# disanda/Deep-GAN-Encoders

Hardware: AMD Instinct MI355X
Metric: encoder-train images/sec (E_align_s2 step, StyleGAN2 FFHQ-1024) (higher is better)
Workload: dtype bf16; 1 GPU; E_align_s2 two-phase step, StyleGAN2-1024 G (train mode) + BE(startf=16, L=9) + LPIPS-VGG16 (seeded stand-in weights), batch 8/GPU; global_batch=8, img_size=1024, parallelism=dp1

## Files before the change

### deep-gan-encoders_amd/_lib.py

```python
import ctypes as C
import os

_HERE = os.path.dirname(os.path.abspath(__file__))
LIB_PATH = os.environ.get("DGE_LIB_PATH", os.path.join(_HERE, "libdge_hip.so"))


class DgeError(RuntimeError):
    pass


class ConvDesc(C.Structure):
    _fields_ = [
        ("x", C.c_void_p), ("w_packed", C.c_void_p), ("y", C.c_void_p), ("addend", C.c_void_p), ("dot_src", C.c_void_p),
        ("in_scale", C.c_void_p), ("in_shift", C.c_void_p), ("out_scale", C.c_void_p),
        ("bias", C.c_void_p), ("noise", C.c_void_p), ("noise_w", C.c_void_p), ("stats", C.c_void_p),
        ("B", C.c_int), ("H", C.c_int), ("W", C.c_int), ("Cin", C.c_int), ("Cout", C.c_int),
        ("ksize", C.c_int), ("up", C.c_int), ("in_s2d", C.c_int), ("noise_batch", C.c_int), ("noise_w_per_channel", C.c_int),
        ("act", C.c_int), ("bias_scale", C.c_float), ("gain", C.c_float), ("add_scale", C.c_float),
        ("dtype", C.c_int), ("in_up2", C.c_int), ("in_relu", C.c_int), ("stats_slots", C.c_int), ("w_layout", C.c_int),
        ("prep", C.c_int), ("prep_gain", C.c_float), ("prep_noise", C.c_void_p), ("prep_ns", C.c_void_p), ("prep_noise_batch", C.c_int),
        ("prep_stats", C.c_void_p), ("mask_relu", C.c_int), ("in_t2d", C.c_int),
        ("rgb_w", C.c_void_p), ("rgb_style", C.c_void_p), ("rgb_bias", C.c_void_p), ("rgb_out", C.c_void_p), ("rgb_wscale", C.c_float),
        ("rgb_skip_y", C.c_int), ("pool_out", C.c_int), ("pool_mask", C.c_void_p),
        ("prefetch_w", C.c_void_p), ("prefetch_ntot", C.c_int), ("prefetch_cin", C.c_int), ("in_bwd_coef", C.c_void_p),
        ("in_bwd_extra", C.c_void_p), ("in_bwd_extra_scale", C.c_float), ("fr_img4", C.c_void_p), ("fr_out", C.c_void_p),
    ]


class ConvPPDesc(C.Structure):
    _fields_ = [
        ("x", C.c_void_p), ("w_pp", C.c_void_p), ("y", C.c_void_p), ("w_bstride", C.c_longlong),
        ("out_scale", C.c_void_p), ("bias", C.c_void_p), ("noise", C.c_void_p), ("noise_w", C.c_void_p),
        ("B", C.c_int), ("H", C.c_int), ("W", C.c_int), ("Cin", C.c_int), ("Cout", C.c_int),
        ("noise_batch", C.c_int), ("noise_w_per_channel", C.c_int), ("act", C.c_int), ("bias_scale", C.c_float), ("gain", C.c_float),
        ("dgrad", C.c_int), ("in_s2d", C.c_int), ("stats_slots", C.c_int), ("prep", C.c_int), ("prep_noise_batch", C.c_int), ("mask_relu", C.c_int),
        ("in_t2d", C.c_int), ("add_scale", C.c_float), ("prep_gain", C.c_float),
        ("dot_src", C.c_void_p), ("addend", C.c_void_p), ("stats", C.c_void_p), ("prep_stats", C.c_void_p), ("prep_noise", C.c_void_p), ("prep_ns", C.c_void_p),
    ]


class DenseLayer(C.Structure):
    _fields_ = [("w", C.c_void_p), ("bias", C.c_void_p), ("I", C.c_int), ("O", C.c_int), ("wscale", C.c_float), ("bscale", C.c_float),
                ("add", C.c_float), ("act", C.c_int), ("gain", C.c_float)]


class S2GradEntry(C.Structure):
    _fields_ = [("P", C.c_void_p), ("st", C.c_void_p), ("d", C.c_void_p), ("s", C.c_void_p), ("bias", C.c_void_p), ("wsq", C.c_void_p),
                ("gs", C.c_void_p), ("wstyle", C.c_void_p),
                ("nslot_p", C.c_int), ("nslot_s", C.c_int), ("in_c", C.c_int), ("out_c", C.c_int), ("row", C.c_int), ("bscale", C.c_float)]


class SumPlanarEntry(C.Structure):
    _fields_ = [("partial", C.c_void_p), ("out", C.c_void_p), ("nslot", C.c_int), ("C", C.c_int), ("NS", C.c_int), ("pad", C.c_int)]


_P, _I, _F = C.c_void_p, C.c_int, C.c_float
SIGNATURES = {
    "dge_conv2d": [C.POINTER(ConvDesc), _P],
    "dge_fir_t2d": [_P, _P, _P, _I, _I, _I, _I, _I, _P],
    "dge_s2_style_grads": [C.POINTER(S2GradEntry), _I, _P, _I, _I, _I, _F, _P],
    "dge_conv_small_supported": [_I, _I, _I, _I, _I, _I, _I, _I],
    "dge_torgb_bwd_prep": [_P, _P, _P, _P, _P, _P, _I, _P, _P, _P, _I, _I, _I, _F, _F, _I, _P],
    "dge_demod_bwd_prep": [_P, _I, _P, _P, _P, _I, _I, _F, _P],
    "dge_sum_slots": [_P, _P, _I, _I, _I, _P],
    "dge_sum_slots_planar": [_P, _P, _I, _I, _I, _P],
    "dge_set_deterministic": [_I],
    "dge_get_deterministic": [],
    "dge_packed_n": [_I],
    "dge_pack_conv_weight": [_P, _P, _I, _I, _I, _I, _I, _F, _P],
    "dge_pack_conv_weights_multi": [_P, _P, _I, _I, _P],
    "dge_pack_desc_bytes": [],
    "dge_weight_sumsq": [_P, _P, _I, _I, _I, _F, _P],
    "dge_linear": [_P, _I, _P, _P, _P, _I, _I, _I, _I, _F, _F, _F, _I, _F, _I, _P],
    "dge_pixelnorm": [_P, _P, _I, _I, _F, _P],
    "dge_truncation": [_P, _P, _P, _I, _I, _I, _F, _I, _I, _P],
    "dge_torgb": [_P, _P, _P, _P, _P, _P, _I, _I, _I, _I, _F, _I, _P],
    "dge_conv_rgb_supported": [_I, _I, _I, _I, _I, _I, _I],
    "dge_conv_in_bwd_supported": [_I, _I, _I, _I, _I, _I, _I],
    "dge_conv_in_bwd_fromrgb_supported": [_I, _I, _I, _I, _I, _I, _I],
    "dge_conv_in_bwd_x_supported": [_I, _I, _I, _I, _I, _I, _I],
    "dge_conv_pool_supported": [_I, _I, _I, _I, _I, _I, _I],
    "dge_rgb_upsample_add": [_P, _P, _I, _I, _I, _P],
    "dge_nchw_to_nhwc": [_P, _P, _I, _I, _I, _I, _I, _P],
    "dge_nhwc_to_nchw": [_P, _P, _I, _I, _I, _I, _P],
    "dge_fromrgb": [_P, _P, _P, _P, _P, _I, _I, _I, _I, _P],
    "dge_fromrgb2": [_P, _P, _P, _P, _P, _P, _I, _I, _I, _I, _P],
    "dge_stats_finalize": [_P, _P, _P, _P, _I, _I, _I, _F, _P],
    "dge_stats_finalize_slots": [_P, _I, _P, _P, _P, _I, _I, _I, _F, _P],
    "dge_blend": [_P, _P, _P, _P, _P, _P, _I, _I, _I, _I, _I, _F, _F, _I, _P],
    "dge_loss_reduce": [_P, _P, _P, _I, _I, _I, _I, _I, _I, _I, _I, _P],
    "dge_crop_pool": [_P, _P, _I, _I, _I, _I, _I, _I, _I, _I, _P],
    "dge_ssim_fwd": [_P, _P, _P, _P, _I, _I, _I, _P],
    "dge_ssim_box7": [_P, _P, _P, _I, _I, _I, _F, _F, _F, _P],
    "dge_ssim_bwd": [_P, _P, _P, _P, _I, _I, _I, _F, _I, _P],
    "dge_space_loss_finalize": [_P, _P, _P, _P, _F, _F, _I, _P],
    "dge_space_loss_bwd": [_P, _P, _P, _P, _P, _I, _I, _I, _I, _I, _I, _I, _I, _F, _F, _I, _P],
    "dge_axpy_scalar": [_P, _P, _P, C.c_long, _F, _I, _P],
    "dge_lreq_adam_multi": [_I, _P, _P, _P, _P, _P, _F, _F, _P, _P, _P],
    "dge_modconv_bwd_prep": [_P, _P, _P, _P, _P, _P, _I, _I, _I, _I, _F, _I, _P],
    "dge_demod_bwd": [_P, _P, _P, _P, _P, _I, _I, _F, _P],
    "dge_linear_t": [_P, _I, _I, _P, _P, _P, _I, _I, _I, _I, _I, _F, _I, _P],
    "dge_torgb_bwd": [_P, _P, _P, _P, _P, _P, _I, _I, _I, _F, _I, _P],
    "dge_up2_bwd": [_P, _P, _I, _I, _I, _P],
    "dge_conv_wgrad": [_P, _P, _P, _P, _P, _I, _I, _I, _I, _I, _I, _I, _P],
    "dge_act_bwd": [_P, _P, _P, _P, _P, _I, _I, _I, _I, _I, _I, _F, _F, _I, _P],
    "dge_in_bwd_coef": [_P, _P, _P, _P, _P, _P, _I, _I, _I, _P],
    "dge_in_bwd_coef_slots": [_P, _I, _P, _P, _P, _P, _P, _I, _I, _I, _P],
    "dge_in_bwd": [_P, _P, _P, _P, _P, _P, _P, _I, _I, _I, _I, _I, _F, _I, _I, _P],
    "dge_chan_sum": [_P, _P, _I, _I, _I, _F, _I, _P],
    "dge_fromrgb_bwd": [_P, _P, _P, _P, _I, _I, _I, _I, _P],
    "dge_head_entry_size": [],
# ... 31 lines not shown
    "dge_upconv_fir": [_P, _P, _P, _P, _P, _P, _I, _P, _I, _P, _F, _F, _I, _I, _I, _I, _I, _I, _I, _P],
    "dge_cbn_affine": [_P, _P, _I, _P, _P, _F, _P, _P, _I, _I, _P],
    "dge_slice_up": [_P, _P, _I, _I, _I, _I, _I, _I, _I, _P],
    "dge_attention": [_P, _P, _P, _P, _I, _I, _I, _I, _I, _I, _P],
    "dge_rgb_tanh": [_P, _P, _I, _I, _I, _I, _P],
    "dge_guided_relu_bwd": [_P, _P, _P, C.c_long, _I, _I, _P],
    "dge_maxpool2_relu_bwd": [_P, _P, _P, _I, _I, _I, _I, _I, _I, _P],
    "dge_maxpool2_bwd_relu": [_P, _P, _P, _P, _I, _I, _I, _I, _I, _P],
    "dge_adaptive_pool7": [_P, _P, _I, _I, _I, _I, _I, _P],
    "dge_adaptive_pool7_bwd": [_P, _P, _I, _I, _I, _I, _I, _P],
    "dge_class_target": [_P, _P, _P, _P, _I, _I, _P],
    "dge_gather_row": [_P, _P, _P, _I, _I, _F, _P],
    "dge_campp_map": [_P, _P, _P, _P, _P, _I, _I, _I, _I, _I, _P],
    "dge_cam_resize": [_P, _P, _P, _I, _I, _I, _I, _I, _P],
    "dge_mask2cam_blocks": [_I],
    "dge_mask2cam": [_P, _P, _P, _P, _P, _P, _P, _I, _I, _P],
    "dge_randn": [_P, _I, _P, _P, _P, _P, C.c_ulonglong, _P, _P],
    "dge_version": [],
    "dge_env_reload": [],
    "dge_blend_pool_mask": [_P, _P, _P, _P, _P, _I, _I, _I, _I, _F, _F, _I, _P],
    "dge_act_bwd_mask": [_P, _P, _P, _P, _P, _I, _I, _I, _I, _I, _F, _F, _I, _P],
    "dge_loss_reduce3": [_P, _P, _P, _I, _I, _I, _I, _P, _I, _P],
    "dge_crop_pool_multi": [_P, _P, _P, _P, _I, _I, _I, _I, _P],
    "dge_space_loss_bwd3": [_P, _P, _P, _P, _P, _I, _I, _I, _P, _P, _P, _P, _I, _P],
    "dge_space_loss_bwd_split": [_P, _P, _P, _P, _P, _I, _I, _I, _P, _P, _P, _P, _I, _P],
    "dge_in_bwd_fromrgb": [_P, _P, _P, _I, _P, _P, _P, _P, _I, _P, _P, _P, _I, _I, _I, _I, _I, _F, _I, _P],
    "dge_in_bwd_fused": [_P, _P, _P, _I, _P, _P, _P, _P, _I, _P, _P, _P, _P, _I, _I, _I, _I, _I, _F, _I, _I, _P],
    "dge_sum_slots_planar_multi": [C.POINTER(SumPlanarEntry), _I, _P],
    "dge_heads_fwd": [_P, _I, _P, _P, _I, _I, _I, _P],
    "dge_conv_pp_supported": [_I, _I, _I, _I, _I, _I],
    "dge_pack_conv_pp": [_P, _P, _I, _I, _F, _P, _P, _F, _I, _I, _P],
    "dge_dense_chain": [_P, _I, C.POINTER(DenseLayer), _I, _P, _I, _I, _I, _F, _P],
    "dge_conv_wgrad_dots": [_P, _P, _P, _P, _P, _P, _P, _I, _I, _I, _I, _I, _I, _I, _P],
    "dge_pack_conv_pp_rows": [_P, _I, _P, _I, _I, _P, _I, _P, _F, _I, _I, _P],
    "dge_conv_pp": [C.POINTER(ConvPPDesc), _P],
    "dge_up_pp_supported": [_I, _I, _I, _I, _I, _I],
    "dge_pack_up_pp": [_P, _P, _I, _I, _P, _P, _F, _I, _P],
    "dge_up_pp": [_P, _P, C.c_longlong, _P, _P, _I, _P, _P, _F, _F, _I, _I, _I, _I, _I, _I, _P],
    "dge_latent_pnorm_fwd": [_P, _P, _P, C.c_long, _I, _P],
    "dge_latent_pnorm_bwd": [_P, _P, _P, _P, C.c_long, _I, _F, _P],
    "dge_wplus_lerp": [_P, _P, _I, _F, _P, _I, _I, _I, _P],
    "dge_wplus_lerp_bwd": [_P, _F, _P, C.c_long, _I, _P],
    "dge_embed_track": [_P, _P, _P, C.c_long, _P, _P, _P, _P, _P, _I, _I, _I, _F, _F, _P],
    "dge_mapping_bwd": [_P, _I, C.POINTER(DenseLayer), _I, _P, _P, _I, _P, _P, _I, _I, _I, _F, _P],
}

_lib = None


def lib():
    global _lib
    if _lib is None:
        if not os.path.exists(LIB_PATH):
            raise DgeError(f"{LIB_PATH} is missing: build it with deep-gan-encoders_amd/csrc/build.sh "
                           "(__graft_entry__.build()). There is no fallback path.")
        _lib = C.CDLL(LIB_PATH)
        for name, args in SIGNATURES.items():
            fn = getattr(_lib, name)
            fn.argtypes = args
            fn.restype = C.c_int
        for name in ("dge_last_error", "dge_last_kernel"):
            getattr(_lib, name).restype = C.c_char_p
            getattr(_lib, name).argtypes = []
        if os.environ.get("DGE_DETERMINISTIC") == "1":
            import torch
            if torch.cuda.is_available() and _lib.dge_set_deterministic(1) != 0:
# ... 12 lines not shown
```

### deep-gan-encoders_amd/autograd_enc_bwd.py

```python
import os

import torch

from . import ops
from .autograd_enc import grads_in_order, heads_layout, linear_backward
from .weight_cache import pack_cache, packed

FUSE_IN_BWD = not os.environ.get("DGE_NO_FUSED_IN_BWD")


def encoder_backward(E, saved, g_w):
    if saved is None:
        raise RuntimeError("encoder forward ran without saved activations")
    cache = pack_cache(E)
    dev = g_w.device
    L = E.layer_count
    B = g_w.shape[0]
    grads = {}
    g_out = fr = None
    later = ops.DeferredSums()
    post = []

    def flush_sums():
        later.flush()
        for f in post:
            f()
        post.clear()
    R = saved["img"].shape[2]
    dt = ops.dtype_of(saved["x0"])
    heads = None
    if saved.get("musig_all") is not None:
        lay = heads_layout(E, B, dev)
        if g_w.stride(2) != 1 or g_w.stride(1) != lay["O"]:
            g_w = g_w.contiguous()
        f32 = dict(dtype=torch.float32, device=dev)
        gms_all, gw_all = torch.empty(lay["total_m"], **f32), torch.empty(lay["total_w"], **f32)
        gb_all = torch.empty(lay["n"] * lay["O"], **f32)
        ops.check(ops.lib().dge_heads_bwd(ops._p(lay["tab"]), lay["n"], lay["max_I"], ops._f32(g_w), g_w.stride(0),
                                          ops._f32(saved["musig_all"]), ops._p(gms_all), ops._p(gw_all), ops._p(gb_all), B, lay["O"],
                                          ops._stream()), "dge_heads_bwd")

        def heads(i, name):
            moff, woff, boff, I = lay["items"][i]
            grads[name + ".weight"] = gw_all[woff:woff + lay["O"] * I].view(lay["O"], I)
            grads[name + ".bias"] = gb_all[boff:boff + lay["O"]]
            return gms_all[moff:moff + B * I].view(B, I)
    for j in range(L - 1, -1, -1):
        blk = E.decode_block[j]
        rec = saved["blocks"][j]
        pre = f"decode_block.{j}."
        Cc, C2 = blk.inputs, blk.outputs
        H = R >> j
        N = H * H
        last = not blk.has_last_conv
        has3 = Cc != C2
        g_w2, g_w1 = g_w[:, 2 * (L - 1 - j)], g_w[:, 2 * (L - 1 - j) + 1]
        if heads is not None:
            gms2, gms1 = heads(2 * j + 1, pre + "inver_mod2"), heads(2 * j, pre + "inver_mod1")
        else:
            gms2 = linear_backward(blk.inver_mod2, g_w2, rec["musig2"], grads, pre + "inver_mod2")
            gms1 = linear_backward(blk.inver_mod1, g_w1, rec["musig1"], grads, pre + "inver_mod1")
        x, x1 = rec["x"], rec["x1"]
        extra, extra_pool, extra_scale = None, False, 1.0
        fuse2 = False
        if not last:
            if g_out is None:
                raise RuntimeError("non-final encoder block without an output gradient")
            red2 = ops.zeros((3 if has3 else 2, C2), dev)
            g_pre2 = ops.act_bwd_mask(g_out, rec["m2"], rec["n2"], scale=0.111 * 0.25, red=red2, planar=True, defer=later)
            grads[pre + "bias_2"] = red2[0].reshape(1, C2, 1, 1)
            grads[pre + "noise_weight_2"] = red2[1].reshape(1, C2, 1, 1)
            gW2 = ops.zeros(tuple(blk.conv_2.weight.shape), dev)
            dots2 = ops.SlotStats(B, Cc, dev)
            fuse2 = FUSE_IN_BWD and ops.conv_in_bwd_supported(B, H, H, C2, Cc, dt) and \
                ops.conv_wgrad_dots(g_pre2, x1, gW2, rec["sc2"], rec["sh2"], blk.conv_2.weight, dots2)
            if not fuse2:
                ops.conv_wgrad(g_pre2, x1, gW2, rec["sc2"], rec["sh2"])
            grads[pre + "conv_2.weight"] = gW2
            if not fuse2:
                g_y2 = ops.conv2d(g_pre2, packed(cache, blk.conv_2, dt, ops.PACK_DGRAD, H), Cc, 3, stats=dots2, dot_src=x1)
            if has3:
                post.append(lambda n=pre + "conv_3.bias", t=red2[2]: grads.__setitem__(n, t * 0.889))
                gW3 = ops.zeros(tuple(blk.conv_3.weight.shape), dev)
                ops.conv_wgrad(g_out, rec["xp"], gW3)
                grads[pre + "conv_3.weight"] = ops.scale_(gW3, 0.889)
                extra = ops.conv2d(g_out, packed(cache, blk.conv_3, dt, ops.PACK_DGRAD), Cc, 1, gain=0.889)
                extra_pool, extra_scale = True, 0.25
            else:
                extra, extra_pool, extra_scale = g_out, True, 0.889 * 0.25
        else:
            if g_out is not None:
                raise RuntimeError("the final encoder block's activation output carries no gradient in E_align")
            g_y2, dots2 = None, None
        coef2 = (dots2, gms2, rec["musig2"], rec["sc2"], rec["sh2"], N)
        red1 = ops.zeros((2, Cc), dev)
        if fuse2:
            redp = ops.SlotStats(B, Cc, dev)
            g_pre1 = ops.conv2d(g_pre2, packed(cache, blk.conv_2, dt, ops.PACK_DGRAD, H), Cc, 3, dot_src=x1,
                                in_bwd=dict(coef=ops.in_bwd_coef(*coef2), noise=rec["n1"].reshape(B, H, H), red=redp))
            ops._sum_planar(redp.buf.view(-1, Cc, 2), red1, later)
        else:
            g_pre1 = ops.in_bwd(g_y2, x1, coef2, noise=rec["n1"], act=True, red=red1, planar=True, defer=later)
        grads[pre + "bias_1"] = red1[0].reshape(1, Cc, 1, 1)
        grads[pre + "noise_weight_1"] = red1[1].reshape(1, Cc, 1, 1)
        gW1 = ops.zeros(tuple(blk.conv_1.weight.shape), dev)
        dots1 = ops.SlotStats(B, Cc, dev)
        fuse_fr = FUSE_IN_BWD and j == 0 and saved.get("img4") is not None and ops.conv_in_bwd_fromrgb_supported(B, H, H, Cc, Cc, dt) and \
            ops.conv_wgrad_dots(g_pre1, x, gW1, rec["sc1"], rec["sh1"], blk.conv_1.weight, dots1)
        fuse_x = FUSE_IN_BWD and not fuse_fr and j > 0 and (extra is None or extra_pool) and ops.conv_in_bwd_x_supported(B, H, H, Cc, Cc, dt) and \
            ops.conv_wgrad_dots(g_pre1, x, gW1, rec["sc1"], rec["sh1"], blk.conv_1.weight, dots1)
        if not (fuse_fr or fuse_x):
            ops.conv_wgrad(g_pre1, x, gW1, rec["sc1"], rec["sh1"])
        grads[pre + "conv_1.weight"] = gW1
        coef1 = (dots1, gms1, rec["musig1"], rec["sc1"], rec["sh1"], N)
        if fuse_fr:
            frh = ops.SlotStats(B, Cc, dev)
            ops.conv2d(g_pre1, packed(cache, blk.conv_1, dt, ops.PACK_DGRAD, H), Cc, 3, dot_src=x, out=x.new_empty((1, 1, 1, 1)),
                       in_bwd=dict(coef=ops.in_bwd_coef(*coef1), fr=frh, img4=saved["img4"], extra=extra if extra_pool else None,
                                   extra_scale=extra_scale))
            fr = ops._sum_planar(frh.buf.view(-1, Cc, 4), torch.empty((4, Cc), dtype=torch.float32, device=dev), later)
        elif fuse_x:
            g_out = ops.conv2d(g_pre1, packed(cache, blk.conv_1, dt, ops.PACK_DGRAD, H), Cc, 3, dot_src=x,
                               in_bwd=dict(coef=ops.in_bwd_coef(*coef1), extra=extra, extra_scale=extra_scale))
        else:
            g_y1 = ops.conv2d(g_pre1, packed(cache, blk.conv_1, dt, ops.PACK_DGRAD, H), Cc, 3, stats=dots1, dot_src=x)
        if fuse_fr or fuse_x:
            pass
        elif j == 0 and Cc <= 512:
            fr = ops.in_bwd_fromrgb(g_y1, x, coef1, saved["img"].float(), extra=extra, extra_pool=extra_pool, extra_scale=extra_scale,
                                    defer=later)
        else:
            g_out = ops.in_bwd(g_y1, x, coef1, extra=extra, extra_pool=extra_pool, extra_scale=extra_scale)
# ... 13 lines not shown
```

### deep-gan-encoders_amd/csrc/capi.hip

```cpp
#include <stdarg.h>
#include <stdio.h>
#include "common.h"
#include "conv_params.h"
#include "../../include/dge_hip.h"

static thread_local char g_err[512] = "";
void dge_set_error(const char* fmt, ...) {
    va_list ap; va_start(ap, fmt); vsnprintf(g_err, sizeof(g_err), fmt, ap); va_end(ap);
}
extern "C" const char* dge_last_error(void) { return g_err; }
static thread_local char g_kernel[160] = "";
void dge_note_kernel(const char* fmt, ...) {
    va_list ap; va_start(ap, fmt); vsnprintf(g_kernel, sizeof(g_kernel), fmt, ap); va_end(ap);
}
extern "C" const char* dge_last_kernel(void) { return g_kernel; }
extern "C" int dge_version(void) { return 100; }

#include <vector>
static std::vector<void (*)(const DgeDet*)>& det_setters() { static std::vector<void (*)(const DgeDet*)> v; return v; }
void dge_det_register(void (*setter)(const DgeDet*)) { det_setters().push_back(setter); }
static DgeDet g_det_host = {0, nullptr, nullptr, 0, 0};
int dge_det_upload_failed = 0;
bool dge_det_fits(long long ndomains, long long nslots, long long L) {
    return !g_det_host.enabled || (ndomains * nslots * L <= g_det_host.ws_floats && ndomains <= (long long)g_det_host.ncounters);
// ... 62 lines not shown
    p.x = d->x; p.w = d->w_packed; p.y = d->y; p.addend = d->addend; p.dot_src = d->dot_src;
    p.in_scale = d->in_scale; p.in_shift = d->in_shift; p.out_scale = d->out_scale;
    p.bias = d->bias; p.noise = d->noise; p.noise_w = d->noise_w; p.stats = d->stats;
    p.B = d->B; p.H = d->H; p.W = d->W; p.Cin = d->Cin; p.Cout = d->Cout;
    p.Ntot_valid = d->up ? 4 * d->Cout : d->Cout;
    p.Ntot = dge_packed_n(p.Ntot_valid);
    p.up = d->up; p.in_s2d = d->in_s2d; p.in_up2 = d->in_up2; p.in_relu = d->in_relu;
    const int OH = d->up ? 2 * d->H : d->H, OW = d->up ? 2 * d->W : d->W;
    p.noise_bstride = d->noise_batch > 1 ? OH * OW : 0;
    p.noise_w_stride = d->noise_w_per_channel ? 1 : 0;
    p.act = d->act; p.bias_scale = d->bias_scale; p.gain = d->gain; p.add_scale = d->add_scale;
    p.tiles_x = p.tiles_y = 0;
    p.w_frag = d->w_layout == 1 ? 1 : 0;
    p.prep = d->prep ? 1 : 0;
    p.mask_relu = d->mask_relu ? 1 : 0;
    p.in_t2d = d->in_t2d ? 1 : 0;
    DGE_CHECK(!d->in_t2d || (d->ksize == 3 && !d->up && !d->in_s2d && !d->in_up2 && !d->in_scale && !d->in_shift && d->w_layout == 0),
              "conv2d: in_t2d is a plain 3x3 launch (no other read mode, no prologue affine, row-major weights)");
    p.prep_gain = d->prep_gain; p.prep_noise = d->prep_noise; p.prep_ns = d->prep_ns; p.prep_stats = d->prep_stats;
    p.prep_noise_bstride = d->prep_noise_batch > 1 ? OH * OW : 0;
    DGE_CHECK(!d->prep || (d->dot_src && d->prep_stats && d->prep_gain > 0.f && !d->up), "conv2d: prep needs dot_src, prep_stats, a positive prep_gain and no up mode");
    DGE_CHECK(!d->prep || !dge_get_deterministic(), "conv2d: the fused tail backward (prep) is not offered in deterministic mode; run dge_modconv_bwd_prep");
    DGE_CHECK(d->w_layout == 0 || d->w_layout == 1, "conv2d: bad w_layout %d", d->w_layout);
    p.stats_slots = d->stats_slots > 0 ? d->stats_slots : 1;
    p.rgb_w = d->rgb_out ? d->rgb_w : nullptr; p.rgb_style = d->rgb_style; p.rgb_bias = d->rgb_bias; p.rgb_out = d->rgb_out;
    p.rgb_wscale = d->rgb_wscale; p.rgb_skip_y = (d->rgb_out && d->rgb_skip_y) ? 1 : 0;
    p.pool_out = d->pool_out ? 1 : 0; p.pool_mask = d->pool_out ? (unsigned*)d->pool_mask : nullptr;
    const bool pf = d->w_layout == 1 && d->prefetch_w && d->prefetch_ntot >= 64 && d->prefetch_ntot % 64 == 0 &&
                    (d->prefetch_cin == 512 || d->prefetch_cin == 256);
    p.pf_w = pf ? d->prefetch_w : nullptr; p.pf_ntot = pf ? d->prefetch_ntot : 0; p.pf_cin = pf ? d->prefetch_cin : 0;
    p.in_coef = d->in_bwd_coef;
    p.in_extra = d->in_bwd_coef ? d->in_bwd_extra : nullptr; p.in_extra_scale = d->in_bwd_extra_scale;
    p.fr_img4 = d->in_bwd_coef ? d->fr_img4 : nullptr; p.fr_out = d->in_bwd_coef ? d->fr_out : nullptr;
    if (d->in_bwd_coef) {
        DGE_CHECK(!dge_get_deterministic(), "conv2d: in_bwd_coef is not offered in deterministic mode; run dge_in_bwd");
        DGE_CHECK(d->ksize == 3 && !d->up && dge_conv_stream_eligible(p, d->dtype, d->ksize), "conv2d: in_bwd_coef is offered where "
                  "dge_conv_in_bwd_supported() says so, with dot_src and prep_stats, without stats / prep");
    }
    if (d->pool_out)
        DGE_CHECK(!d->up && dge_conv_pool_ok(p, d->dtype, d->ksize), "conv2d: the pooled epilogue is offered where dge_conv_pool_supported() "
                  "says so (conv_2 of the first encoder blocks on the streaming kernel)");
    if (d->rgb_out) {
        DGE_CHECK(d->rgb_w && d->rgb_style && d->rgb_bias, "conv2d: rgb_out needs rgb_w, rgb_style, rgb_bias");
        DGE_CHECK(dge_conv_rgb_ok(p, d->dtype, d->ksize), "conv2d: the fused toRGB is offered where dge_conv_rgb_supported() says so "
                  "(bf16 3x3 32 -> 32 launches of the streaming kernel)");
    }
    return dge_conv_launch(p, d->dtype, d->ksize, s);
}

extern "C" int dge_conv_pool_supported(int B, int H, int W, int Cin, int Cout, int ksize, int dtype) {
    ConvParams p = {};
    p.B = B; p.H = H; p.W = W; p.Cin = Cin; p.Cout = Cout; p.Ntot_valid = Cout; p.Ntot = dge_packed_n(Cout);
    p.in_shift = (const float*)16; p.noise_w_stride = 1;
    return dge_conv_pool_ok(p, dtype, ksize) ? 1 : 0;
}

extern "C" int dge_conv_in_bwd_supported(int B, int H, int W, int Cin, int Cout, int ksize, int dtype) {
    ConvParams p = {};
    p.B = B; p.H = H; p.W = W; p.Cin = Cin; p.Cout = Cout; p.Ntot_valid = Cout; p.Ntot = dge_packed_n(Cout);
    p.dot_src = (const void*)16; p.prep_stats = (float*)16; p.in_coef = (const float*)16;
    return (ksize == 3 && !dge_get_deterministic() && dge_conv_stream_eligible(p, dtype, ksize)) ? 1 : 0;
}
extern "C" int dge_conv_in_bwd_x_supported(int B, int H, int W, int Cin, int Cout, int ksize, int dtype) {
    ConvParams p = {};
    p.B = B; p.H = H; p.W = W; p.Cin = Cin; p.Cout = Cout; p.Ntot_valid = Cout; p.Ntot = dge_packed_n(Cout);
    p.dot_src = (const void*)16; p.in_coef = (const float*)16;
    return (ksize == 3 && !dge_get_deterministic() && dge_conv_stream_eligible(p, dtype, ksize)) ? 1 : 0;
}
extern "C" int dge_conv_in_bwd_fromrgb_supported(int B, int H, int W, int Cin, int Cout, int ksize, int dtype) {
    ConvParams p = {};
    p.B = B; p.H = H; p.W = W; p.Cin = Cin; p.Cout = Cout; p.Ntot_valid = Cout; p.Ntot = dge_packed_n(Cout);
    p.dot_src = (const void*)16; p.in_coef = (const float*)16; p.fr_img4 = (const float*)16; p.fr_out = (float*)16;
    return (ksize == 3 && !dge_get_deterministic() && dge_conv_stream_eligible(p, dtype, ksize)) ? 1 : 0;
}

extern "C" int dge_conv_rgb_supported(int B, int H, int W, int Cin, int Cout, int ksize, int dtype) {
    ConvParams p = {};
    p.B = B; p.H = H; p.W = W; p.Cin = Cin; p.Cout = Cout; p.Ntot_valid = Cout; p.Ntot = dge_packed_n(Cout);
    return dge_conv_rgb_ok(p, dtype, ksize) ? 1 : 0;
}

__global__ void sum_slots_kernel(const float* __restrict__ partial, float* __restrict__ out, int nslot, int n, int accumulate) {
    const int i = blockIdx.x * blockDim.x + threadIdx.x;
    if (i >= n) return;
    float s = 0.f;
    int k = 0;
    for (; k + 8 <= nslot; k += 8) {
        float v[8];
#pragma unroll
        for (int j = 0; j < 8; j++) v[j] = partial[(size_t)(k + j) * n + i];
#pragma unroll
        for (int j = 0; j < 8; j++) s += v[j];
    }
    for (; k < nslot; k++) s += partial[(size_t)k * n + i];
// ... 61 lines not shown
```

### deep-gan-encoders_amd/csrc/conv_params.h

```cpp
#pragma once
#include <hip/hip_runtime.h>

struct ConvParams {
    const void* x;
    const void* w;
    void* y;
    const void* addend;
    const void* dot_src;
    const float* in_scale;
    const float* in_shift;
    const float* out_scale;
    const float* bias;
    const float* noise;
    const float* noise_w;
    float* stats;
    int stats_slots;
    int B, H, W, Cin, Cout;
    int Ntot;
    int Ntot_valid;
    int up;
    int in_s2d;
    int in_relu;
    int in_up2;
    int noise_bstride;
    int noise_w_stride;
    int act;
    float bias_scale, gain, add_scale;
    int tiles_x, tiles_y;
    int dbg;
    int w_frag;
    int prep;
    float prep_gain;
    const float* prep_noise;
    const float* prep_ns;
    int prep_noise_bstride;
    float* prep_stats;
    int mask_relu;
    int in_t2d;
    const float* rgb_w;
    const float* rgb_style;
    const float* rgb_bias;
    float* rgb_out;
    float rgb_wscale;
    int rgb_skip_y;
    int pool_out;
    unsigned* pool_mask;
    const void* pf_w;
    int pf_ntot, pf_cin;
    const float* in_coef;
    const void* in_extra; float in_extra_scale; const float* fr_img4; float* fr_out;
};

int dge_conv_launch(const ConvParams& p, int dtype, int ksize, hipStream_t s);
extern "C" int dge_conv_ntile(int ntot);

bool dge_conv_stream_eligible(const ConvParams& p, int dtype, int ksize);
int dge_conv_stream_launch(const ConvParams& p, hipStream_t s);
bool dge_conv_rgb_ok(const ConvParams& p, int dtype, int ksize);
bool dge_conv_pool_ok(const ConvParams& p, int dtype, int ksize);
bool dge_conv_small_shape_ok(int H, int W, int cin, int ntot, int ksize, int in_s2d, int in_up2, int dtype);
int dge_conv_small_launch(const ConvParams& p, hipStream_t s);
bool dge_conv_pw_eligible(const ConvParams& p, int dtype, int ksize);
int dge_conv_pw_launch(const ConvParams& p, hipStream_t s);
```

### deep-gan-encoders_amd/csrc/conv_stream.hip

```cpp
#include <type_traits>
#include "common.h"
#include <stdlib.h>
#include "conv_params.h"

namespace {

typedef __attribute__((ext_vector_type(4))) unsigned rsrc_t;
#define DGE_LDS " lds\n\t"

__device__ __forceinline__ unsigned rfl(unsigned v) { return __builtin_amdgcn_readfirstlane(v); }
__device__ __forceinline__ unsigned lds_off(const void* p) {
    return (unsigned)(size_t)(const __attribute__((address_space(3))) unsigned char*)p;
}
constexpr int ilog2(int v) { return v <= 1 ? 0 : 1 + ilog2(v >> 1); }

__device__ __forceinline__ rsrc_t make_rsrc(unsigned long long base, unsigned bytes) {
    rsrc_t r;
    r[0] = rfl((unsigned)base); r[1] = rfl((unsigned)(base >> 32) & 0xffffu); r[2] = rfl(bytes); r[3] = 0x00020000u;
    return r;
}

#define DGE_P(off) "buffer_load_dwordx4 %1, %3, 0 offen offset:" #off " lds\n\t"
#define DGE_PB(off) "buffer_load_dwordx4 %4, %3, 0 offen offset:" #off " lds\n\t"
#define DGE_M0 "s_mov_b32 m0, %2\n\ts_nop 0\n\t"
// ... 9 lines not shown
        if (wave == 0) asm volatile(DGE_M0 DGE_P(0) : "=&s"(keep) : "v"(voff), "s"(m0v), "s"(rs) : "memory");
        else asm volatile(DGE_M0 DGE_MASK(0xf) DGE_P(1024) DGE_UNMASK : "=&s"(keep) : "v"(voff), "s"(m0v), "s"(rs) : "memory");
    } else if constexpr (CIN == 32 && TEAM == 1) {
        asm volatile(DGE_M0 DGE_P(0) DGE_P(1024) DGE_MASK(0xff) DGE_P(2048) DGE_UNMASK : "=&s"(keep) : "v"(voff), "s"(m0v), "s"(rs) : "memory");
    } else if constexpr (CIN == 32 && TEAM == 2) {
        if (wave == 0) asm volatile(DGE_M0 DGE_P(0) DGE_MASK(0xff) DGE_P(2048) DGE_UNMASK : "=&s"(keep) : "v"(voff), "s"(m0v), "s"(rs) : "memory");
        else asm volatile(DGE_M0 DGE_P(1024) "s_mov_b32 m0, %5\n\ts_nop 0\n\tbuffer_load_dwordx4 %1, %4, 0 offen lds"
                          : "=&s"(keep) : "v"(voff), "s"(m0v), "s"(rs), "s"(rs_null), "s"(m0_dummy) : "memory");
    } else if constexpr (CIN == 64 && TEAM == 1) {
        asm volatile(DGE_M0 DGE_P(0) DGE_PB(1024) DGE_P(2048) DGE_PB(3072)
                     "s_mov_b32 m0, %6\n\t" DGE_MASK(0xffff) "buffer_load_dwordx4 %5, %3, 0 offen lds\n\t" DGE_UNMASK
                     : "=&s"(keep) : "v"(voff), "s"(m0v), "s"(rs), "v"(voff_b), "v"(voff_c), "s"(m0v + 4096u) : "memory");
    } else {
        if (wave == 0)
            asm volatile(DGE_M0 DGE_P(0) DGE_P(2048)
                         "s_mov_b32 m0, %5\n\t" DGE_MASK(0xffff) "buffer_load_dwordx4 %4, %3, 0 offen lds\n\t" DGE_UNMASK
                         : "=&s"(keep) : "v"(voff), "s"(m0v), "s"(rs), "v"(voff_c), "s"(m0v + 4096u) : "memory");
        else
            asm volatile(DGE_M0 DGE_P(1024) DGE_P(3072) "s_mov_b32 m0, %5\n\ts_nop 0\n\tbuffer_load_dwordx4 %1, %4, 0 offen lds"
                         : "=&s"(keep) : "v"(voff_b), "s"(m0v), "s"(rs), "s"(rs_null), "s"(m0_dummy) : "memory");
    }
}
__device__ __forceinline__ void dma_piece(unsigned voff, rsrc_t rs, unsigned m0v) {
    asm volatile("s_mov_b32 m0, %1\n\ts_nop 0\n\tbuffer_load_dwordx4 %0, %2, 0 offen lds" : : "v"(voff), "s"(m0v), "s"(rs) : "memory");
}
template <int NP> __device__ __forceinline__ void dma_dot(unsigned voff, unsigned voff1, rsrc_t rs, unsigned m0v) {
    if constexpr (NP == 1)
        asm volatile("s_mov_b32 m0, %1\n\ts_nop 0\n\tbuffer_load_dwordx4 %0, %2, 0 offen lds" : : "v"(voff), "s"(m0v), "s"(rs) : "memory");
    else
        asm volatile("s_mov_b32 m0, %1\n\ts_nop 0\n\tbuffer_load_dwordx4 %0, %2, 0 offen lds\n\t"
                     "buffer_load_dwordx4 %3, %2, 0 offen offset:1024 lds" : : "v"(voff), "s"(m0v), "s"(rs), "v"(voff1) : "memory");
}

enum { FL_GEN = 0, FL_ENC = 1, FL_ENC_STATS = 2, FL_DOT = 3, FL_DOT_PREP = 4, FL_GEN_RGB = 5, FL_ENC_POOL = 6, FL_DOT_IN = 7, FL_DOT_FR = 8, FL_DOT_INX = 9 };

template <int CIN, int COUT, int FL>
struct SC {
    static constexpr int PXB = CIN * 2, CH = PXB / 16, LOGCH = ilog2(CH), KS = CIN / 16;
    static constexpr int TEAM = COUT == 64 ? 2 : 1;
    static constexpr int TPW = 4 / TEAM;
    static constexpr int MT = COUT / 32 > 0 ? COUT / 32 : 1;
    static constexpr int MTW = MT / TEAM;
    static constexpr int HW = 34, RB = HW * PXB;
    static constexpr int PIECES = (RB + 1023) / 1024;
    static constexpr bool PREP = FL == FL_DOT_PREP, RGB = FL == FL_GEN_RGB, POOL = FL == FL_ENC_POOL, FRB = FL == FL_DOT_FR, INX = FL == FL_DOT_INX, INB = FL == FL_DOT_IN || FRB || INX;
    static_assert(!RGB || COUT == 32 || (COUT == 64 && TEAM == 2), "fused toRGB: 32 output channels per wave, one wave or a 2-wave team per pixel");
    static constexpr bool DOT = FL == FL_DOT || PREP || INB, STATS = FL == FL_ENC_STATS, ENC = FL == FL_ENC || FL == FL_ENC_STATS || POOL;
    static constexpr bool NOISE = !DOT || PREP || (INB && !FRB && !INX);
    static constexpr int NR = 6;
    static constexpr int dot_depth(int nr) { for (int d = 4; d >= 1; d--) if (d <= nr - 3 && nr % (d + 1) == 0) return d; return 1; }
    static constexpr int D = DOT ? dot_depth(6) : 2;
    static constexpr int DR = DOT ? D + 1 : NR;
    static_assert(NR % DR == 0, "dot ring period");
    static constexpr int CPB = COUT * 2;
    static constexpr int CW = COUT / TEAM >= 32 ? 32 : 16;
    static constexpr int DCH = CW * MTW * 2 / 16;
    static constexpr int LOGDCH = ilog2(DCH);
    static constexpr int DROWB = 32 * DCH * 16, DPIECES = DROWB / 1024;
    static_assert(!DOT || MTW == 1, "data-gradient mode: one M tile per wave");
    static constexpr int XPW = TEAM == 2 ? (PIECES + 1) / 2 : PIECES;
    static constexpr int LPR = XPW + (DOT ? DPIECES : 0) + (FRB ? 2 : 0) + (INX ? 1 : 0);
    static constexpr int X_OFF = 0;
    static constexpr int XRING = NR * RB;
    static constexpr int N_OFF = (XRING + 1023) / 1024 * 1024;
    static constexpr int NRING = NOISE ? 2048 : 0;
    static_assert(NR <= 8, "a noise piece holds 8 rows");
    static constexpr int D_OFF = N_OFF + TEAM * NRING;
    static constexpr int DRING = DOT ? DR * DROWB : 0;
    static constexpr int E_OFF = D_OFF + TEAM * DRING;
    static constexpr int ERING = FRB ? 2 * DR * 512 : (INX ? DR * 1024 : 0);
    static_assert(!INX || (CIN == COUT && CIN >= 32), "block-input flavour: 32 -> 32, 64 -> 64");
    static_assert(!FRB || (CIN == 16 && COUT == 16 && TEAM == 1), "FromRGB reduction flavour: 16 -> 16");
    static constexpr int T_OFF = E_OFF + TEAM * ERING;
    static constexpr int TBYTES = 32 * MTW * 16 * 4;
    static constexpr int DUMMY_OFF = T_OFF + TEAM * TBYTES;
    static constexpr int RGBX_OFF = DUMMY_OFF + (TEAM == 2 ? 1024 : 0);
    static constexpr int LDS_BYTES = RGBX_OFF + (RGB && TEAM == 2 ? 1024 : 0);
    static constexpr int NEED = 4 * 9 * KS * MTW + 32 * MTW + 16 + (ENC ? 16 * MTW : 0) + (STATS || DOT ? 32 * MTW : 0) + (DOT ? 16 : 0) + (PREP ? 16 : 0) + (RGB ? 11 : 0) + (POOL ? 20 * MTW : 0) + 36;
    static constexpr int WPE = ((PREP || INB) && CIN == 64) ? 1 : (NEED <= 128 ? 4 : (NEED <= 168 ? 3 : 2));
    static_assert(D <= NR - 3, "the slot of the row being fetched must be dead");
    static_assert((D - 1) * LPR + 1 < 64, "vmcnt range");
};

template <int LOGC> __device__ __forceinline__ int chunk_swz(int px) { return (px >> (4 - LOGC)) & ((1 << LOGC) - 1); }

template <int CW> __device__ __forceinline__ int chan_of_row(int m) {
    const int j = m >> 3, k = (m >> 2) & 1, i = m & 3;
    if (CW == 16) return j < 2 ? 8 * k + 4 * j + i : -1;
    return 16 * (j >> 1) + 8 * k + 4 * (j & 1) + i;
}

template <int CIN, int COUT, int FL>
__global__ __launch_bounds__((64 * SC<CIN, COUT, FL>::TEAM * SC<CIN, COUT, FL>::TPW), (SC<CIN, COUT, FL>::WPE))
void conv_stream_kernel(ConvParams p, int nstrips, int nseg, int seg_rows, int njobs, int jobs_per_xcd) {
    using C = SC<CIN, COUT, FL>;
    extern __shared__ __attribute__((aligned(1024))) unsigned char lds_all[];
#ifdef DGE_SC_TIMING
    const long long tj0 = __builtin_readcyclecounter();
#endif
    const int lane = threadIdx.x & 63;
    const int wid = (int)rfl(threadIdx.x >> 6);
    const int team = wid / C::TEAM;
    const int wave = wid % C::TEAM;
    unsigned char* __restrict__ lds = lds_all + team * C::LDS_BYTES;
    const unsigned lds0 = lds_off(lds_all) + team * C::LDS_BYTES;
    const int n31 = lane & 31, kh = lane >> 5;

    int job = ((blockIdx.x & 7) * jobs_per_xcd + (blockIdx.x >> 3)) * C::TPW + team;
    if ((blockIdx.x >> 3) >= jobs_per_xcd || job >= njobs) return;
    const int strip = job % nstrips; job /= nstrips;
    const int seg = job % nseg;
    const int b = job / nseg;
    const int x0 = strip * 32;
    const int r0 = seg * seg_rows;
// ... 10 lines not shown
    const unsigned long long DOTb = C::DOT ? (unsigned long long)p.dot_src + (unsigned long long)b * p.H * yrow_bytes : Xb;

    unsigned voff, voff_b = 0, voff_c = 0;
    {
        const int px = lane >> C::LOGCH, cs = lane & (C::CH - 1);
        const int gx = x0 - 1 + px;
        voff = (unsigned)(gx * C::PXB + ((cs ^ chunk_swz<C::LOGCH>(px)) << 4));
        if constexpr (CIN == 64) {
            voff_b = (unsigned)(gx * C::PXB + ((cs ^ chunk_swz<C::LOGCH>(px + 8)) << 4));
            voff_c = voff + 4096;
        }
    }
    const unsigned nvoff = (unsigned)(((lane >> 3) * p.W + x0 + (lane & 7) * 4) * 4);
    unsigned dvoff = 0, dvoff1 = 0;
    if constexpr (C::DOT) {
        const int px = lane >> C::LOGDCH, cs = lane & (C::DCH - 1);
        const int chunk0 = wave * 4;
        dvoff = (unsigned)((x0 + px) * C::CPB + ((chunk0 + (cs ^ chunk_swz<C::LOGDCH>(px))) << 4));
        constexpr int PPP = 64 / C::DCH;
        dvoff1 = (unsigned)((x0 + px + PPP) * C::CPB + ((chunk0 + (cs ^ chunk_swz<C::LOGDCH>(px + PPP))) << 4)) - 1024u;
    }
    const rsrc_t rs_null = make_rsrc(Xb, 0);
    const unsigned exrow_bytes = (C::FRB || C::INX) ? (unsigned)(p.W >> 1) * C::CPB : 0u, imrow_bytes = C::FRB ? (unsigned)p.W * 16u : 0u;
    const unsigned long long EXb = ((C::FRB || C::INX) && p.in_extra) ? (unsigned long long)p.in_extra + (unsigned long long)b * (p.H >> 1) * exrow_bytes : Xb;
    const unsigned long long IMb = C::FRB ? (unsigned long long)p.fr_img4 + (unsigned long long)b * p.H * imrow_bytes : Xb;
    const unsigned evoff = C::INX ? (unsigned)(((x0 >> 1) + (lane >> 2)) * C::CPB + wave * 64 + (((lane & 3) ^ chunk_swz<2>(lane >> 2)) << 4))
                                  : (unsigned)((x0 >> 1) * 32 + (lane & 31) * 16);
    const unsigned ivoff = (unsigned)((x0 + (lane & 31)) * 16);

    unsigned long long xptr = Xb + (unsigned long long)(long long)(r0 - 1) * xrow_bytes;
    unsigned long long dptr = DOTb + (unsigned long long)(long long)(r0 - 2) * yrow_bytes;
    auto issue = [&](int h, int slot, int slot_d) {
        const int gy = r0 - 1 + h;
        const bool xv = (unsigned)gy < (unsigned)p.H && h <= rows + 1;
        const rsrc_t rx = make_rsrc(xptr, xv ? xrow_bytes : 0u);
        xptr += xrow_bytes;
        const unsigned m0x = lds0 + C::X_OFF + slot * C::RB;
        dma_row<CIN, C::TEAM>(wave, voff, voff_b, voff_c, rx, rs_null, m0x, lds0 + C::DUMMY_OFF);
        const bool ov = h >= 2 && h <= rows + 1;
        if constexpr (C::DOT) {
            const rsrc_t rd = make_rsrc(dptr, ov ? yrow_bytes : 0u);
            dptr += yrow_bytes;
            dma_dot<C::DPIECES>(dvoff, dvoff1, rd, lds0 + C::D_OFF + wave * C::DRING + slot_d * C::DROWB);
        }
        if constexpr (C::INX) {
            const int oy = gy - 1;
            const rsrc_t re = make_rsrc(EXb + (unsigned long long)(ov ? (oy >> 1) : 0) * exrow_bytes, (ov && p.in_extra) ? exrow_bytes : 0u);
            dma_piece(evoff, re, lds0 + C::E_OFF + wave * C::ERING + slot_d * 1024);
        }
        if constexpr (C::FRB) {
            const int oy = gy - 1;
            const rsrc_t re = make_rsrc(EXb + (unsigned long long)(ov ? (oy >> 1) : 0) * exrow_bytes, (ov && p.in_extra) ? exrow_bytes : 0u);
            const rsrc_t ri = make_rsrc(IMb + (unsigned long long)(ov ? oy : 0) * imrow_bytes, ov ? imrow_bytes : 0u);
            unsigned long long keep;
            asm volatile(DGE_MASK(0xffffffff) "s_mov_b32 m0, %2\n\ts_nop 0\n\tbuffer_load_dwordx4 %1, %3, 0 offen lds\n\t"
                         "s_mov_b32 m0, %4\n\ts_nop 0\n\tbuffer_load_dwordx4 %5, %6, 0 offen lds\n\t" DGE_UNMASK
                         : "=&s"(keep) : "v"(evoff), "s"(lds0 + C::E_OFF + slot_d * 512), "s"(re), "s"(lds0 + C::E_OFF + C::DR * 512 + slot_d * 512), "v"(ivoff), "s"(ri) : "memory");
        }
    };
    auto issue_noise = [&](int q, unsigned buf_off) {
        const int gy = r0 + q;
        const bool v = nzsrc != nullptr && gy < p.H && q < rows;
        const rsrc_t rn = make_rsrc(NZb + (unsigned long long)(v ? gy : 0) * nzrow_bytes, v ? (unsigned)(p.H - gy) * nzrow_bytes : 0u);
        dma_piece(nvoff, rn, lds0 + C::N_OFF + wave * C::NRING + buf_off);
    };
    asm volatile("s_waitcnt vmcnt(0)" ::: "memory");
    if constexpr (C::NOISE) issue_noise(0, 0u);
    StaticFor<C::D + 2>::run([&](auto hc) { constexpr int h = decltype(hc)::value; issue(h, h % C::NR, (h + C::NR - 2) % C::NR % C::DR); });

    uint4 wf[C::MTW][9][C::KS];
    float* __restrict__ TT = (float*)(lds + C::T_OFF + wave * C::TBYTES);
    {
        const bf16_t* __restrict__ Wp = (const bf16_t*)p.w;
        float sc[C::KS][8], rt[C::KS][8];
#pragma unroll
        for (int ks = 0; ks < C::KS; ks++) {
            const int k0 = ks * 16 + kh * 8;
#pragma unroll
            for (int e = 0; e < 8; e++) {
                sc[ks][e] = p.in_scale ? p.in_scale[b * CIN + k0 + e] : 1.f;
                const float sh = (C::ENC && p.in_shift) ? p.in_shift[b * CIN + k0 + e] : 0.f;
                rt[ks][e] = sc[ks][e] != 0.f ? sh / sc[ks][e] : 0.f;
            }
        }
#pragma unroll
        for (int mt = 0; mt < C::MTW; mt++) {
            const int cl = chan_of_row<C::CW>(n31);
            const int o = (wave * C::MTW + mt) * 32 + cl;
            const bool ov = cl >= 0 && o < COUT;
            float osc = p.gain;
            if (!C::DOT && p.out_scale && ov) osc *= p.out_scale[b * COUT + o];
            if (C::INB && ov) osc *= p.in_coef[((size_t)b * COUT + o) * 3];
            const int oc = ov ? o : 0;
            float c_bias = (!C::DOT && p.bias) ? p.bias[oc] : 0.f;
            float c_nw = (C::NOISE && p.noise) ? p.noise_w[oc * p.noise_w_stride] : 0.f;
            float c_osc = (C::DOT && !C::INB && p.out_scale) ? p.out_scale[b * COUT + oc] : 1.f;
            float c_in1 = 0.f, c_in2 = 0.f;
            if constexpr (C::INB) { c_in1 = p.in_coef[((size_t)b * COUT + oc) * 3 + 1]; c_in2 = p.in_coef[((size_t)b * COUT + oc) * 3 + 2]; }
            float tall = 0.f, tleft = 0.f, tright = 0.f;
            {
// ... 120 lines not shown

    const int gx = x0 + n31;
    const bool pv = gx < p.W;
    const unsigned yoff = (unsigned)gx * C::CPB + (unsigned)(wave * C::MTW * 32 * 2) + kh * 16;
    const bool pool_lane = C::POOL && (n31 & 1) == 0 && pv;
    const unsigned py_voff = pool_lane ? (unsigned)(gx >> 1) * C::CPB + (unsigned)(wave * C::MTW * 64) + kh * 16 : 0x80000000u;
    const unsigned pm_voff = pool_lane ? ((unsigned)(gx >> 1) * (COUT / 8) + (unsigned)(wave * C::MTW * 4) + kh) * 4u : 0x80000000u;
    const unsigned pool_px = C::POOL ? (unsigned)(p.H >> 1) * (unsigned)(p.W >> 1) : 0u;
    const __amdgpu_buffer_rsrc_t rs_pool = __builtin_amdgcn_make_buffer_rsrc((unsigned char*)p.y + (size_t)b * pool_px * C::CPB, 0, (int)(pool_px * C::CPB), 0x00020000);
    const __amdgpu_buffer_rsrc_t rs_mask = __builtin_amdgcn_make_buffer_rsrc((C::POOL && p.pool_mask) ? (unsigned char*)p.pool_mask + (size_t)b * pool_px * (COUT / 8) * 4 : (unsigned char*)p.y, 0,
                                                                               (C::POOL && p.pool_mask) ? (int)(pool_px * (COUT / 8) * 4) : 0, 0x00020000);

    float s0[C::MTW][(C::STATS || C::DOT) ? 16 : 1], s1[C::MTW][(C::STATS || C::DOT) ? 16 : 1], s2[(C::PREP || C::INB) ? 16 : 1];
    if constexpr (C::STATS || C::DOT) {
#pragma unroll
        for (int mt = 0; mt < C::MTW; mt++)
#pragma unroll
            for (int r = 0; r < 16; r++) { s0[mt][r] = 0.f; s1[mt][r] = 0.f; }
    }
    if constexpr (C::PREP || C::INB) {
#pragma unroll
        for (int r = 0; r < 16; r++) s2[r] = 0.f;
    }
    float prow[C::POOL ? C::MTW : 1][C::POOL ? 16 : 1];
    unsigned psign[C::POOL ? C::MTW : 1];
    const float pg_pos = p.prep_gain, pg_neg = 0.2f * p.prep_gain, pz_pos = 1.f / p.prep_gain, pz_neg = 1.f / (0.2f * p.prep_gain);
    const float pns = (C::PREP && p.prep_noise && p.prep_ns) ? p.prep_ns[0] : 0.f;
    const float fr_es = (C::FRB || C::INX) ? p.in_extra_scale : 0.f;

#define DGE_T(k)
    auto step = [&](auto ic, int s, unsigned npar) {
        constexpr int I = decltype(ic)::value;
        DGE_T(0);
        constexpr int NAFTER = (C::D - 1) * C::LPR + ((C::NOISE && I >= 1 && I <= C::D - 1) ? 1 : 0);
        asm volatile("s_waitcnt vmcnt(%0)" :: "i"(NAFTER) : "memory");
        if constexpr (C::RGB && C::TEAM == 2) asm volatile("s_waitcnt lgkmcnt(0)" ::: "memory");
        if constexpr (C::TEAM == 2) __builtin_amdgcn_s_barrier();
        if constexpr (C::RGB && C::TEAM == 2) { if (wave == 0 && s > 0) rgb_flush(s - 1); }
        DGE_T(1);
        if constexpr (C::NOISE && I == 0) issue_noise(s + C::NR, npar ^ 1024u);
        issue(s + 2 + C::D, (I + 2 + C::D) % C::NR, (I + C::D) % C::DR);
        DGE_T(2);

        const int gy = r0 + s;
        constexpr int NQ = 9 * C::KS;
        constexpr int PF = NQ < 6 ? NQ : 6;
        auto frag_addr = [&](auto qc) {
            constexpr int q = decltype(qc)::value;
            constexpr int tap = q / C::KS, ks = q % C::KS, dy = tap / 3, dx = tap % 3;
            return loff[dx][ks] + (unsigned)(((I + dy) % C::NR) * C::RB);
        };
        float nz = 0.f;
        if constexpr (C::NOISE) nz = lds_f(nzoff + npar + I * 128);
        uint4 bq[PF];
        StaticFor<PF>::run([&](auto qc) { bq[decltype(qc)::value] = lds_u4(frag_addr(qc)); });
        f32x16_t acc[C::MTW];
        StaticFor<NQ>::run([&](auto qc) {
            constexpr int q = decltype(qc)::value;
            constexpr int tap = q / C::KS, ks = q % C::KS;
            const bf16x8_t bf = *(const bf16x8_t*)&bq[q % PF];
#pragma unroll
            for (int mt = 0; mt < C::MTW; mt++) {
                acc[mt] = __builtin_amdgcn_mfma_f32_32x32x16_bf16(*(const bf16x8_t*)&wf[mt][tap][ks], bf, q == 0 ? ((C::DOT && !C::INB) ? zero16 : biasv[mt]) : acc[mt], 0, 0, 0);
            }
            if constexpr (q + PF < NQ) bq[q % PF] = lds_u4(frag_addr(std::integral_constant<int, q + PF>{}));
        });

        __builtin_amdgcn_sched_group_barrier(0x100, PF + (C::NOISE ? 1 : 0), 0);
        StaticFor<NQ - PF>::run([&](auto) {
            __builtin_amdgcn_sched_group_barrier(0x008, C::MTW, 0);
            __builtin_amdgcn_sched_group_barrier(0x100, 1, 0);
        });
        __builtin_amdgcn_sched_group_barrier(0x008, PF * C::MTW, 0);
// ... 130 lines not shown
            if constexpr (C::RGB) {
                f32x16_t t = __builtin_amdgcn_mfma_f32_32x32x16_bf16(*(const bf16x8_t*)&rgbA[0], *(const bf16x8_t*)&o0, zero16, 0, 0, 0);
                t = __builtin_amdgcn_mfma_f32_32x32x16_bf16(*(const bf16x8_t*)&rgbA[1], *(const bf16x8_t*)&o1, t, 0, 0, 0);
                if constexpr (C::TEAM == 2) {
                    if (wave == 0) { rgbh[0] = t[0] + t[4] + rgbb[0]; rgbh[1] = t[1] + t[5] + rgbb[1]; rgbh[2] = t[2] + t[6] + rgbb[2]; }
                    else if (kh == 0) {
                        const unsigned a = lds0 + C::RGBX_OFF + (unsigned)(s & 1) * 384 + n31 * 4;
                        *(lds_wfp)(a) = t[0] + t[4]; *(lds_wfp)(a + 128) = t[1] + t[5]; *(lds_wfp)(a + 256) = t[2] + t[6];
                    }
                } else if (kh == 0 && pv) {
                    float* __restrict__ ro = p.rgb_out + ((size_t)b * 3 * p.H + gy) * p.W + gx;
                    const size_t plane = (size_t)p.H * p.W;
                    ro[0] = t[0] + t[4] + rgbb[0]; ro[plane] = t[1] + t[5] + rgbb[1]; ro[2 * plane] = t[2] + t[6] + rgbb[2];
                }
                if (p.rgb_skip_y) continue;
            }
            if (full_strip) {
                *(uint4*)dst = o0;
                if constexpr (NREG == 16) *(uint4*)(dst + 32) = o1;
            } else if (pv) {
                *(uint4*)dst = o0;
                if constexpr (NREG == 16) *(uint4*)(dst + 32) = o1;
            }
        }
        DGE_T(4);
    };

#ifdef DGE_SC_TIMING
    const int tjob_id = ((blockIdx.x & 7) * jobs_per_xcd + (blockIdx.x >> 3)) * C::TPW + team;
    __builtin_amdgcn_sched_barrier(0);
    const long long tj1 = __builtin_readcyclecounter();
    __builtin_amdgcn_sched_barrier(0);
#endif
    unsigned npar = 0;
    for (int s0_ = 0; s0_ < rows; s0_ += C::NR, npar ^= 1024u) {
        bool done = false;
        StaticFor<C::NR>::run([&](auto ic) {
            constexpr int I = decltype(ic)::value;
            if (!done) {
                if ((C::POOL && (I & 1)) || s0_ + I < rows) step(ic, s0_ + I, npar);
                else done = true;
            }
        });
    }
    if constexpr (C::RGB && C::TEAM == 2) {
        asm volatile("s_waitcnt lgkmcnt(0)" ::: "memory");
        __builtin_amdgcn_s_barrier();
        if (wave == 0 && rows > 0) rgb_flush(rows - 1);
    }
    asm volatile("s_waitcnt vmcnt(0)" ::: "memory");
#ifdef DGE_SC_TIMING
    if (lane == 0 && wave == 0) {
        long long* tl = (long long*)p.y + (size_t)tjob_id * 4;
        tl[0] = tj0; tl[1] = tj1; tl[2] = __builtin_readcyclecounter(); tl[3] = ((long long)rows << 40) | (long long)(__builtin_amdgcn_s_memrealtime() & 0xffffffffffll);
    }
#endif

    if constexpr (C::FRB) {
        float va = 0.f, vc = 0.f;
#pragma unroll
        for (int r = 0; r < 16; r++) {
            float a = pv ? s0[0][r] : 0.f, c = pv ? s1[0][r] : 0.f;
#pragma unroll
            for (int m = 1; m < 32; m <<= 1) { a += __shfl_xor(a, m, 64); c += __shfl_xor(c, m, 64); }
            if (n31 == r) { va = a; vc = c; }
        }
// ... 37 lines not shown
                }
            }
            if (!C::PREP && !C::INB && det && det_arrive_wave(b, nseg * nstrips * C::TEAM)) {
                for (int idx = lane; idx < COUT * 2; idx += 64)
                    p.stats[(size_t)b * COUT * 2 + idx] = det_sum(b, nseg * nstrips, COUT * 2, idx);
            }
        }
    }
}

template <int CIN, int COUT, int FL>
int launch_stream(const ConvParams& p0, hipStream_t s) {
    using C = SC<CIN, COUT, FL>;
    ConvParams p = p0;
    auto kern = conv_stream_kernel<CIN, COUT, FL>;
    static int caps[16] = {0};
    int dev = 0;
    (void)hipGetDevice(&dev);
    int& cap = caps[dev >= 0 && dev < 16 ? dev : 0];
    if (!cap) {
        (void)hipFuncSetAttribute((const void*)kern, hipFuncAttributeMaxDynamicSharedMemorySize, C::LDS_BYTES * C::TPW);
        int occ = 0, ncu = 256;
        (void)hipDeviceGetAttribute(&ncu, hipDeviceAttributeMultiprocessorCount, dev);
        if (hipOccupancyMaxActiveBlocksPerMultiprocessor(&occ, (const void*)kern, 64 * C::TEAM * C::TPW, C::LDS_BYTES * C::TPW) != hipSuccess || occ < 1) occ = 1;
        cap = occ * ncu * C::TPW;
    }
    const int nstrips = (p.W + 31) / 32;
    int nseg = cap / (p.B * nstrips);
    if (dge_env().stream_nseg > 0) nseg = dge_env().stream_nseg;
    int maxseg = p.H / 16; if (maxseg < 1) maxseg = 1;
    if (nseg > maxseg) nseg = maxseg;
    if (nseg < 1) nseg = 1;
    int seg_rows = (p.H + nseg - 1) / nseg;
    if (C::POOL) seg_rows += seg_rows & 1;
    nseg = (p.H + seg_rows - 1) / seg_rows;
    const int njobs = p.B * nstrips * nseg;
    const int nwg = (njobs + C::TPW - 1) / C::TPW;
    const int jobs_per_xcd = (nwg + 7) / 8;
    const char* fl = FL == FL_GEN ? "gen" : (FL == FL_ENC ? "enc" : (FL == FL_ENC_STATS ? "enc_stats" : (FL == FL_DOT ? "dot" : (FL == FL_DOT_PREP ? "dot_prep" : (FL == FL_GEN_RGB ? "gen_rgb" : (FL == FL_DOT_IN ? "dot_in" : (FL == FL_DOT_FR ? "dot_fromrgb" : (FL == FL_DOT_INX ? "dot_inx" : "enc_pool"))))))));
    dge_note_kernel("conv_stream<bf16,%d,%d,%s>", CIN, COUT, fl);
    hipLaunchKernelGGL(kern, dim3((unsigned)(jobs_per_xcd * 8)), dim3(64 * C::TEAM * C::TPW), C::LDS_BYTES * C::TPW, s, p, nstrips, nseg, seg_rows, njobs, jobs_per_xcd);
    DGE_LAUNCH_CHECK("conv_stream");
    return 0;
}

template <int CIN, int COUT>
int launch_flavour(const ConvParams& p, hipStream_t s) {
    if (p.in_coef && p.fr_out) {
        if constexpr (CIN == 16 && COUT == 16) return launch_stream<CIN, COUT, FL_DOT_FR>(p, s);
        dge_set_error("conv_stream: the FromRGB reduction epilogue is built for 16 -> 16 only");
        return -1;
    }
    if (p.in_coef && !p.prep_stats) {
        if constexpr (CIN == COUT && CIN >= 32) return launch_stream<CIN, COUT, FL_DOT_INX>(p, s);
        dge_set_error("conv_stream: the block-input instance-norm backward epilogue is built for 32 -> 32 and 64 -> 64 only");
        return -1;
    }
    if (p.in_coef) {
        if constexpr ((CIN == 32 && COUT == 16) || (CIN == 64 && COUT == 32)) return launch_stream<CIN, COUT, FL_DOT_IN>(p, s);
        dge_set_error("conv_stream: the instance-norm backward epilogue is built for 32 -> 16 and 64 -> 32 only");
        return -1;
    }
    if (p.dot_src) {
        if constexpr (CIN == COUT && CIN >= 32) {
            if (p.prep) return launch_stream<CIN, COUT, FL_DOT_PREP>(p, s);
        }
        if (p.prep) { dge_set_error("conv_stream: the fused tail backward is built for 32->32 and 64->64 only"); return -1; }
        return launch_stream<CIN, COUT, FL_DOT>(p, s);
    }
    const bool enc = p.stats || p.in_shift || (p.noise && p.noise_w_stride != 0);
    if (p.rgb_out) {
        if constexpr ((CIN == 32 && COUT == 32) || (CIN == 64 && COUT == 64)) { if (!enc) return launch_stream<CIN, COUT, FL_GEN_RGB>(p, s); }
        dge_set_error("conv_stream: the fused toRGB is built for the generator flavour of 32 -> 32 and 64 -> 64 only");
        return -1;
    }
    if (p.pool_out) {
        if constexpr ((CIN == 16 && COUT == 32) || (CIN == 32 && COUT == 64)) { if (!p.stats) return launch_stream<CIN, COUT, FL_ENC_POOL>(p, s); }
        dge_set_error("conv_stream: the pooled epilogue is built for the encoder's 16 -> 32 and 32 -> 64 layers without statistics");
        return -1;
    }
    if constexpr (CIN == 64) {
        if (enc) { dge_set_error("conv_stream: encoder flavour with Cin = 64 is not built"); return -1; }
    } else {
        if (p.stats) return launch_stream<CIN, COUT, FL_ENC_STATS>(p, s);
        if (enc) return launch_stream<CIN, COUT, FL_ENC>(p, s);
    }
    return launch_stream<CIN, COUT, FL_GEN>(p, s);
}

}

bool dge_conv_stream_eligible(const ConvParams& p, int dtype, int ksize) {
    if (dtype != DGE_BF16 || ksize != 3 || p.up || p.in_s2d || p.in_up2 || p.in_relu || p.addend || p.mask_relu || p.in_t2d) return false;
    if (!(p.Cin == 16 || p.Cin == 32 || p.Cin == 64) || !(p.Cout == 16 || p.Cout == 32 || p.Cout == 64)) return false;
    if (p.W % 4 != 0 || p.W < 64 || p.H < 32) return false;
    if ((long)p.H * p.W < 128L * 128) return false;
    {
        const long px = (long)p.B * p.H * p.W;
        const bool enc = p.stats || p.in_shift || (p.noise && p.noise_w_stride != 0);
        if (!dge_env().force_stream) {
            if (!p.dot_src && px < (enc ? (1L << 20) : (1L << 18))) return false;
            if (p.dot_src && px < (1L << 16)) return false;
        }
    }
    if ((long)p.W * p.Cin * 2 >= (1L << 31) || (long)p.H * p.W * 64 * 2 >= (1L << 40)) return false;
    if (p.dot_src && !p.stats && !p.in_coef) return false;
    if (p.in_coef && !p.fr_out && p.prep_stats && !(p.dot_src && !p.prep && !p.stats && ((p.Cin == 32 && p.Cout == 16) || (p.Cin == 64 && p.Cout == 32)))) return false;
    if (p.in_coef && !p.fr_out && !p.prep_stats && !(p.dot_src && !p.prep && !p.stats && p.Cin == p.Cout && p.Cin >= 32 && p.H % 2 == 0 && p.W % 2 == 0)) return false;
    if (p.fr_out && !(p.in_coef && p.dot_src && p.fr_img4 && !p.prep && !p.stats && p.Cin == 16 && p.Cout == 16 && p.H % 2 == 0 && p.W % 2 == 0)) return false;
    if (p.prep && !(p.Cin == p.Cout && p.Cin >= 32)) return false;
    if (p.Cin == 64 && !p.dot_src && (p.stats || p.in_shift || (p.noise && p.noise_w_stride != 0))) return false;
    if (p.dot_src && (p.bias || p.noise || p.in_shift || p.act != DGE_ACT_NONE)) return false;
    if (p.noise && p.noise_w == nullptr) return false;
    if (dge_env().no_stream) return false;
    return true;
}

bool dge_conv_pool_ok(const ConvParams& p, int dtype, int ksize) {
    return ((p.Cin == 16 && p.Cout == 32) || (p.Cin == 32 && p.Cout == 64)) && !p.dot_src && !p.stats && !p.rgb_out && p.H % 2 == 0 && p.W % 2 == 0 &&
           dge_conv_stream_eligible(p, dtype, ksize);
}

bool dge_conv_rgb_ok(const ConvParams& p, int dtype, int ksize) {
    return ((p.Cin == 32 && p.Cout == 32) || (p.Cin == 64 && p.Cout == 64)) && !p.dot_src && !p.stats && !p.in_shift && !(p.noise && p.noise_w_stride != 0) &&
           dge_conv_stream_eligible(p, dtype, ksize);
}

int dge_conv_stream_launch(const ConvParams& p, hipStream_t s) {
#define GO(CI, CO) if (p.Cin == CI && p.Cout == CO) return launch_flavour<CI, CO>(p, s)
#ifdef DGE_SC_ONLY
#define GO2(...) GO(__VA_ARGS__)
    GO2(DGE_SC_ONLY);
#undef GO2
#else
    GO(16, 16); GO(16, 32); GO(16, 64); GO(32, 16); GO(32, 32); GO(32, 64); GO(64, 16); GO(64, 32); GO(64, 64);
#endif
#undef GO
    dge_set_error("conv_stream: unsupported channel configuration %d -> %d", p.Cin, p.Cout);
    return -1;
}
```

### deep-gan-encoders_amd/csrc/enc_bwd_kernels.hip

```cpp
#include <stdlib.h>
#include "common.h"
#include "../../include/dge_hip.h"

template <int NTAP>
__device__ __forceinline__ void wgrad_flush(const f32x16_t (&acc)[NTAP], float* smem, float* __restrict__ dW, int o0, int i0,
                                            int Co, int Ci, int tid, int lane, int wave) {
    float* red = smem;
    float* stage = smem + 4096;
#pragma unroll
    for (int t = 0; t < NTAP; t++) {
        __syncthreads();
#pragma unroll
        for (int r = 0; r < 16; r++) red[wave * 1024 + r * 64 + lane] = acc[t][r];
        __syncthreads();
#pragma unroll
        for (int q = 0; q < 4; q++) {
            const int e = tid + q * 256;
            const int r = e >> 6, ln = e & 63;
            const int ol = (r & 3) + 8 * (r >> 2) + 4 * (ln >> 5), il = ln & 31;
            stage[(ol * 32 + il) * NTAP + t] = (red[e] + red[1024 + e]) + (red[2048 + e] + red[3072 + e]);
        }
    }
    __syncthreads();
    const int ni = (Ci - i0 < 32 ? Ci - i0 : 32) * NTAP;
// ... 289 lines not shown
                                                       float* __restrict__ red_out, int H, int W, int C, int pool, float scale, float slope) {
    constexpr int EP = Elem<T>::PER16;
    __shared__ float red[256 * NS * EP];
    const int b = blockIdx.y;
    const int cpt = C / EP, ppi = 256 / cpt;
    const int chunk = threadIdx.x % cpt, slot = threadIdx.x / cpt;
    const int HW = H * W, UW = pool ? W / 2 : W, UHW = pool ? HW / 4 : HW;
    const float raw_w = pool ? 0.25f : 1.f;
    float s[NS][EP];
#pragma unroll
    for (int k = 0; k < NS; k++)
#pragma unroll
        for (int e = 0; e < EP; e++) s[k][e] = 0.f;
    for (int p0 = blockIdx.x * ppi; p0 < HW; p0 += gridDim.x * ppi) {
        const int p = p0 + slot;
        if (slot < ppi && p < HW) {
            const int q = pool ? (p / W / 2) * UW + (p % W) / 2 : p;
            float g[EP], av[EP];
            unpack16(*(const uint4*)(gup + ((size_t)b * UHW + q) * C + chunk * EP), g, (T*)nullptr);
            unpack16(*(const uint4*)(a + ((size_t)b * HW + p) * C + chunk * EP), av, (T*)nullptr);
            const float nz = noise ? noise[(size_t)b * HW + p] : 0.f;
#pragma unroll
            for (int e = 0; e < EP; e++) {
                if constexpr (NS == 3) s[2][e] += raw_w * g[e];
                g[e] = scale * g[e] * (av[e] > 0.f ? 1.f : slope);
                s[0][e] += g[e]; s[1][e] += g[e] * nz;
            }
            *(uint4*)(gpre + ((size_t)b * HW + p) * C + chunk * EP) = pack16(g, (T*)nullptr);
        }
    }
    if (red_out) block_chan_flush<EP, NS>(s, cpt, ppi, red_out + (size_t)b * C * NS, C, red);
}

template <typename T, int NS>
__global__ __launch_bounds__(256) void act_bwd_mask_kernel(const T* __restrict__ gup, const unsigned* __restrict__ mask,
                                                            const float* __restrict__ noise, T* __restrict__ gpre,
                                                            float* __restrict__ red_out, int H, int W, int C, float scale, float slope) {
    constexpr int EP = Elem<T>::PER16;
    __shared__ float red[256 * NS * EP];
    const int b = blockIdx.y;
    const int cpt = C / EP, ppi = 256 / cpt;
    const int chunk = threadIdx.x % cpt, slot = threadIdx.x / cpt;
    const int UW = W / 2, UHW = (H / 2) * UW, HW = H * W;
    float s[NS][EP];
#pragma unroll
    for (int k = 0; k < NS; k++)
#pragma unroll
        for (int e = 0; e < EP; e++) s[k][e] = 0.f;
    const int stride = gridDim.x * ppi;
    for (int q0 = blockIdx.x * ppi; q0 < UHW; q0 += 2 * stride) {
        const int qq[2] = {q0 + slot, q0 + slot + stride};
        bool ok[2]; uint4 gv[2]; unsigned mv[2]; int p00[2]; float nzv[2][4];
#pragma unroll
        for (int h = 0; h < 2; h++) {
            ok[h] = slot < ppi && qq[h] < UHW;
            gv[h] = make_uint4(0, 0, 0, 0); mv[h] = 0; p00[h] = 0;
#pragma unroll
            for (int c4 = 0; c4 < 4; c4++) nzv[h][c4] = 0.f;
            if (ok[h]) {
                gv[h] = *(const uint4*)(gup + ((size_t)b * UHW + qq[h]) * C + chunk * EP);
                mv[h] = mask[((size_t)b * UHW + qq[h]) * cpt + chunk];
                const int oy = qq[h] / UW, ox = qq[h] - oy * UW;
                p00[h] = (2 * oy) * W + 2 * ox;
                if (noise) {
#pragma unroll
                    for (int c4 = 0; c4 < 4; c4++) nzv[h][c4] = noise[(size_t)b * HW + p00[h] + (c4 >> 1) * W + (c4 & 1)];
                }
            }
        }
#pragma unroll
        for (int h = 0; h < 2; h++) {
            if (!ok[h]) continue;
            float g[EP];
            unpack16(gv[h], g, (T*)nullptr);
            const unsigned m = mv[h];
#pragma unroll
            for (int e = 0; e < EP; e++) { if constexpr (NS == 3) s[2][e] += g[e]; g[e] *= scale; }
#pragma unroll
            for (int c4 = 0; c4 < 4; c4++) {
                const int p = p00[h] + (c4 >> 1) * W + (c4 & 1);
                const float nz = nzv[h][c4];
                float o[EP];
#pragma unroll
                for (int e = 0; e < EP; e++) {
                    o[e] = g[e] * (((m >> (c4 * EP + e)) & 1u) ? 1.f : slope);
                    s[0][e] += o[e]; s[1][e] += o[e] * nz;
                }
                *(uint4*)(gpre + ((size_t)b * HW + p) * C + chunk * EP) = pack16(o, (T*)nullptr);
            }
        }
    }
    if (red_out) block_chan_flush<EP, NS>(s, cpt, ppi, red_out + (size_t)b * C * NS, C, red);
}

__global__ void in_bwd_coef_kernel(const float* __restrict__ dots, const float* __restrict__ gms, const float* __restrict__ musig,
                                   const float* __restrict__ sc, const float* __restrict__ sh, float* __restrict__ coef,
                                   int B, int C, float inv_n, int nslot) {
    const int idx = blockIdx.x * blockDim.x + threadIdx.x;
    if (idx >= B * C) return;
    const int b = idx / C, c = idx % C;
    const float r = sc[idx], s = sh[idx];
    float S2 = 0.f, S1 = 0.f;
    if (dots) {
        const float2 ss = sum_slot_pairs(dots + (size_t)idx * 2, (size_t)B * C * 2, nslot);
        S2 = ss.x; S1 = ss.y;
    }
    const float m1 = S1 * inv_n, m2 = (r * S2 + s * S1) * inv_n;
    const float mu = musig[(size_t)b * 2 * C + c], sg = musig[(size_t)b * 2 * C + C + c];
    const float gmu = gms ? gms[(size_t)b * 2 * C + c] : 0.f, gsg = gms ? gms[(size_t)b * 2 * C + C + c] : 0.f;
    const float k = sg > 0.f ? gsg * inv_n / sg : 0.f;
    coef[(size_t)idx * 3 + 0] = r;
    coef[(size_t)idx * 3 + 1] = -r * r * m2 + k;
    coef[(size_t)idx * 3 + 2] = -r * m1 - r * m2 * s + gmu * inv_n - k * mu;
}

struct InCoefSrc { const float* dots; const float* gms; const float* musig; const float* sc; const float* sh; int nslot, B; float inv_n; };
template <typename T, bool FR>
__global__ __launch_bounds__(256) void in_bwd_kernel(const T* __restrict__ gy, const T* __restrict__ X, const float* __restrict__ coef,
                                                      const T* __restrict__ extra, const float* __restrict__ noise,
                                                      T* __restrict__ gout, float* __restrict__ red_out, int H, int W, int C,
                                                      int extra_pool, float extra_scale, int act, InCoefSrc cs,
// ... 240 lines not shown
        float s = 0.f;
#pragma unroll
        for (int j = 0; j < 16; j++) s += part[j][lane];
        gms_all[e.moff + (size_t)b * e.I + k] = s;
    }
}
__global__ void head_bwd_param_kernel(const HeadEntry* __restrict__ tab, const float* __restrict__ g, int ldg,
                                      const float* __restrict__ musig_all, float* __restrict__ gw_all, float* __restrict__ gb_all,
                                      int B, int O) {
    const HeadEntry e = tab[blockIdx.y];
    const int total = O * e.I;
    for (int idx = blockIdx.x * 256 + threadIdx.x; idx < total; idx += gridDim.x * 256) {
        const int o = idx / e.I, i = idx - o * e.I;
        float s = 0.f, sb = 0.f;
        for (int b = 0; b < B; b++) {
            const float gv = g[(size_t)b * ldg + e.gcol + o];
            s += gv * musig_all[e.moff + (size_t)b * e.I + i]; sb += gv;
        }
        gw_all[e.woff + idx] = s;
        if (i == 0) gb_all[e.boff + o] = sb;
    }
}

#define CHAN_OK(C, ep) ((C) % (ep) == 0 && (C) / (ep) <= 256 && 256 % ((C) / (ep)) == 0)

int dge_wgrad_dma_try(const void* g, const void* x, const float* sc, const float* sh, float* dw, int B, int H, int W, int cout, int cin,
                      const float* wdot, float* dots, int dots_slots, hipStream_t s);
extern "C" int dge_conv_wgrad_dots(const void* g, const void* x, const float* in_scale, const float* in_shift, float* dw, const float* w,
                                   float* dots, int dots_slots, int B, int H, int W, int cout, int cin, int dtype, hipStream_t s) {
    DGE_CHECK(g && x && dw && w && dots && in_scale && in_shift && dots_slots >= 1, "conv_wgrad_dots: null tensor");
    if (dtype != DGE_BF16) return 1;
    return dge_wgrad_dma_try(g, x, in_scale, in_shift, dw, B, H, W, cout, cin, w, dots, dots_slots, s);
}
extern "C" int dge_conv_wgrad(const void* g, const void* x, const float* in_scale, const float* in_shift, float* dw, int B, int H,
                              int W, int cout, int cin, int ksize, int dtype, hipStream_t s) {
    DGE_CHECK(ksize == 1 || ksize == 3, "conv_wgrad: ksize %d unsupported", ksize);
    const int ep = dtype == DGE_BF16 ? 8 : 4;
    DGE_CHECK(cout % ep == 0 && cin % ep == 0, "conv_wgrad: channels must be multiples of %d", ep);
    DGE_CHECK((in_scale == nullptr) == (in_shift == nullptr), "conv_wgrad: in_scale and in_shift go together");
    if (dtype == DGE_BF16 && ksize == 3) {
        const int r = dge_wgrad_dma_try(g, x, in_scale, in_shift, dw, B, H, W, cout, cin, nullptr, nullptr, 1, s);
        if (r <= 0) return r;
    }
    const bool tall = dtype == DGE_BF16 && H >= 16 && !dge_env().wgrad_th8;
    const int tx = (W + 15) / 16, ty = tall ? (H + 15) / 16 : (H + 7) / 8;
    const int ntiles = tx * ty * B;
    const int noi = ((cout + 31) / 32) * ((cin + 31) / 32);
    int groups = 512 / noi; if (groups < 1) groups = 1;
    if (dge_env().wgrad_groups > 0) groups = dge_env().wgrad_groups;
    if (groups > ntiles) groups = ntiles;
    dim3 grid(noi, groups);
    if (dtype == DGE_BF16) dge_note_kernel("conv_wgrad_tr<%d,%d>", ksize, tall ? 16 : 8);
    else dge_note_kernel("conv_wgrad<f32,%d>", ksize);
#define WG(T, KS) hipLaunchKernelGGL((conv_wgrad_kernel<T, KS>), grid, dim3(256), 0, s, (const T*)g, (const T*)x, in_scale, in_shift, dw, B, H, W, cout, cin, tx, ty, groups)
    if (dtype == DGE_BF16) {
#define WT(KS, TH) hipLaunchKernelGGL((conv_wgrad_tr_kernel<KS, TH>), grid, dim3(256), 0, s, (const bf16_t*)g, (const bf16_t*)x, in_scale, in_shift, dw, B, H, W, cout, cin, tx, ty, groups)
        if (ksize == 3) { if (tall) WT(3, 16); else WT(3, 8); }
        else { if (tall) WT(1, 16); else WT(1, 8); }
#undef WT
    }
    else { if (ksize == 3) WG(float, 3); else WG(float, 1); }
#undef WG
    DGE_LAUNCH_CHECK("conv_wgrad");
    return 0;
}

// ... 17 lines not shown
    return 0;
}

extern "C" int dge_head_entry_size(void) { return (int)sizeof(HeadEntry); }
extern "C" int dge_heads_bwd(const void* dev_entries, int n, int max_I, const float* g, int ldg, const float* musig_all, float* gms_all,
                             float* gw_all, float* gb_all, int B, int O, hipStream_t s) {
    DGE_CHECK(n >= 1 && n <= 65535 && B >= 1 && B <= 65535 && O >= 1 && max_I >= 1, "heads_bwd: bad sizes");
    hipLaunchKernelGGL(head_bwd_data_kernel, dim3((max_I + 63) / 64, B, n), dim3(1024), 0, s, (const HeadEntry*)dev_entries, g, ldg, gms_all, O);
    hipLaunchKernelGGL(head_bwd_param_kernel, dim3(64, n), dim3(256), 0, s, (const HeadEntry*)dev_entries, g, ldg, musig_all, gw_all,
                       gb_all, B, O);
    DGE_LAUNCH_CHECK("heads_bwd");
    return 0;
}

extern "C" int dge_act_bwd(const void* gup, const void* a, const float* noise, void* gpre, float* red, int red_cols, int B, int H,
                           int W, int C, int pool, float scale, float slope, int dtype, hipStream_t s) {
    const int ep = dtype == DGE_BF16 ? 8 : 4;
    DGE_CHECK(CHAN_OK(C, ep), "act_bwd: unsupported channel count %d", C);
    DGE_CHECK(red_cols == 2 || red_cols == 3, "act_bwd: red_cols must be 2 or 3 (got %d)", red_cols);
    dim3 grid(dge_stream_grid(H * W, 256 / (C / ep), B), B);
#define AB(T, NS) hipLaunchKernelGGL((act_bwd_kernel<T, NS>), grid, dim3(256), 0, s, (const T*)gup, (const T*)a, noise, (T*)gpre, red, H, W, C, pool, scale, slope)
    if (dtype == DGE_BF16) { if (red_cols == 3) AB(bf16_t, 3); else AB(bf16_t, 2); }
    else { if (red_cols == 3) AB(float, 3); else AB(float, 2); }
#undef AB
    DGE_LAUNCH_CHECK("act_bwd");
    return 0;
}

extern "C" int dge_act_bwd_mask(const void* gup, const unsigned* mask, const float* noise, void* gpre, float* red, int red_cols, int B, int H,
                                int W, int C, float scale, float slope, int dtype, hipStream_t s) {
    const int ep = dtype == DGE_BF16 ? 8 : 4;
    DGE_CHECK(CHAN_OK(C, ep) && H % 2 == 0 && W % 2 == 0 && mask, "act_bwd_mask: unsupported shape (C %d, %d x %d)", C, H, W);
    DGE_CHECK(red_cols == 2 || red_cols == 3, "act_bwd_mask: red_cols must be 2 or 3 (got %d)", red_cols);
    dim3 grid(dge_stream_grid(H * W / 4, 256 / (C / ep), B), B);
#define AB(T, NS) hipLaunchKernelGGL((act_bwd_mask_kernel<T, NS>), grid, dim3(256), 0, s, (const T*)gup, mask, noise, (T*)gpre, red, H, W, C, scale, slope)
    if (dtype == DGE_BF16) { if (red_cols == 3) AB(bf16_t, 3); else AB(bf16_t, 2); }
    else { if (red_cols == 3) AB(float, 3); else AB(float, 2); }
#undef AB
    DGE_LAUNCH_CHECK("act_bwd_mask");
    return 0;
}

extern "C" int dge_in_bwd_coef_slots(const float* dots, int nslot, const float* gms, const float* musig, const float* sc,
                                     const float* sh, float* coef, int B, int C, int npix, hipStream_t s) {
    DGE_CHECK(nslot >= 1, "in_bwd_coef: nslot %d", nslot);
    hipLaunchKernelGGL(in_bwd_coef_kernel, dim3((B * C + 63) / 64), dim3(64), 0, s, dots, gms, musig, sc, sh, coef, B, C, 1.0f / (float)npix, nslot);
    DGE_LAUNCH_CHECK("in_bwd_coef");
    return 0;
}
extern "C" int dge_in_bwd_coef(const float* dots, const float* gms, const float* musig, const float* sc, const float* sh,
                               float* coef, int B, int C, int npix, hipStream_t s) {
    return dge_in_bwd_coef_slots(dots, 1, gms, musig, sc, sh, coef, B, C, npix, s);
}

static int in_bwd_launch(const void* gy, const void* x, const float* coef, const InCoefSrc& cs, const void* extra, const float* noise, void* gout,
                         float* red, int B, int H, int W, int C, int extra_pool, float extra_scale, int act, int dtype, hipStream_t s,
                         const float* img = nullptr, float* fr_out = nullptr) {
    const int ep = dtype == DGE_BF16 ? 8 : 4;
    DGE_CHECK(CHAN_OK(C, ep), "in_bwd: unsupported channel count %d", C);
    dim3 grid(dge_stream_grid(H * W, 256 / (C / ep), B), B);
#define DGE_IB(T, FR) hipLaunchKernelGGL((in_bwd_kernel<T, FR>), grid, dim3(256), 0, s, (const T*)gy, (const T*)x, coef, (const T*)extra, noise, (T*)gout, red, H, W, C, extra_pool, extra_scale, act, cs, img, fr_out)
    if (img) { if (dtype == DGE_BF16) DGE_IB(bf16_t, true); else DGE_IB(float, true); }
    else { if (dtype == DGE_BF16) DGE_IB(bf16_t, false); else DGE_IB(float, false); }
#undef DGE_IB
    DGE_LAUNCH_CHECK("in_bwd");
    return 0;
}
extern "C" int dge_in_bwd(const void* gy, const void* x, const float* coef, const void* extra, const float* noise, void* gout,
// ... 69 lines not shown
```

### deep-gan-encoders_amd/csrc/wgrad_dma.hip

```cpp
#include <stdlib.h>
#include <type_traits>
#include "common.h"
#include "../../include/dge_hip.h"

namespace {

typedef __attribute__((ext_vector_type(4))) unsigned rsrc_t;
typedef short v4s_t __attribute__((ext_vector_type(4)));
typedef __attribute__((address_space(3))) v4s_t* lds_v4s_ptr;

__device__ __forceinline__ unsigned rfl(unsigned v) { return __builtin_amdgcn_readfirstlane(v); }
__device__ __forceinline__ unsigned lds_off(const void* p) {
    return (unsigned)(size_t)(const __attribute__((address_space(3))) unsigned char*)p;
}
__device__ __forceinline__ rsrc_t make_rsrc(unsigned long long base, unsigned bytes) {
    rsrc_t r;
    r[0] = rfl((unsigned)base); r[1] = rfl((unsigned)(base >> 32) & 0xffffu); r[2] = rfl(bytes); r[3] = 0x00020000u;
    return r;
}
__device__ __forceinline__ void dma16(unsigned voff, rsrc_t rs, unsigned m0v) {
    asm volatile("s_mov_b32 m0, %1\n\ts_nop 0\n\tbuffer_load_dwordx4 %0, %2, 0 offen lds" : : "v"(voff), "s"(m0v), "s"(rs) : "memory");
}
constexpr unsigned DEAD = 0x7fffffffu;

template <int TH_, int GP_, int XP_, int NW_, int NS_>
struct WCfg {
    static constexpr int TH = TH_, GP = GP_, XP = XP_, NW = NW_, NS = NS_;
    static constexpr int TW = 16, HH = TH + 2, HWD = TW + 2;
    static constexpr int GBYTES = TH * TW * GP;
    static constexpr int XBYTES = ((HH * HWD + 4) * XP + 1023) / 1024 * 1024;
    static constexpr int NGP = GBYTES / 1024, NXP = XBYTES / 1024, NP = NGP + NXP;
    static constexpr int PW = (NP + NW - 1) / NW;
    static constexpr int STAGE = GBYTES + XBYTES;
    static constexpr int RING = NS * STAGE;
    static constexpr int FLUSH = (NW * 1024 + 1024 * 9) * 4;
    static constexpr int MAIN = RING > FLUSH ? RING : FLUSH;
    static constexpr int GTAB_OFF = MAIN, TAB_OFF = GTAB_OFF + 9 * 32 * 4;
    static constexpr int RW = TH / NW;
    static_assert(TH % NW == 0 && (NS - 2) * PW <= 63 && GBYTES % 1024 == 0 && NS >= 2 && NS <= 5, "configuration");
    static int lds_bytes() { return TAB_OFF + 64 * 4; }
};

#ifdef DGE_WG_TIMING
__device__ long long wg_tlog[64 * 6];
#define DGE_WT(k) do { __builtin_amdgcn_sched_barrier(0); const long long t_ = __builtin_readcyclecounter(); __builtin_amdgcn_sched_barrier(0); \
                       if (tlogon && t - t_begin >= 8 && t - t_begin < 40) wg_tlog[(t - t_begin - 8) * 6 + k] = t_; } while (0)
#else
#define DGE_WT(k)
#endif

template <class C>
__global__ __launch_bounds__(C::NW * 64, 2) void wgrad_dma_kernel(const bf16_t* __restrict__ g, const bf16_t* __restrict__ X,
                                                                const float* __restrict__ sc, const float* __restrict__ sh,
                                                                float* __restrict__ dW, int B, int H, int W, int Co, int Ci,
                                                                int tiles_x, int tiles_y, int per_group, int gps,
                                                                const float* __restrict__ Wdot, float* __restrict__ dots, int dots_slots) {
    constexpr int TH = C::TH, GP = C::GP, XP = C::XP, NW = C::NW, NS = C::NS, NT = NW * 64;
    extern __shared__ __attribute__((aligned(1024))) unsigned char lds[];
    float* gtab = (float*)(lds + C::GTAB_OFF);
    float* sctab = (float*)(lds + C::TAB_OFF);
    float* ktab = sctab + 32;
    const int tid = threadIdx.x, lane = tid & 63;
    const int wave = __builtin_amdgcn_readfirstlane(tid >> 6);
    const int n_it = (Ci + 31) / 32;
    const int noi = gridDim.x, lin = blockIdx.x + noi * blockIdx.y;
    int grp_id = blockIdx.y, oi = blockIdx.x;
    if (!(gridDim.y & 7)) { const int slot = lin >> 3; grp_id = (slot / noi) * 8 + (lin & 7); oi = slot % noi; }
    const int o0 = (oi / n_it) * 32, i0 = (oi % n_it) * 32;
    const int tps = tiles_x * tiles_y;
    if (grp_id >= B * gps) return;
    const int smp = grp_id / gps, part = grp_id - smp * gps;
    const int t_begin = smp * tps + part * per_group;
    const int t_end = t_begin + per_group < (smp + 1) * tps ? t_begin + per_group : (smp + 1) * tps;
    if (t_begin >= t_end) return;
    const bool aff = sc != nullptr;
    if (aff && tid < 32) {
        const int ch = i0 + tid;
        sctab[tid] = ch < Ci ? sc[smp * Ci + ch] : 1.f;
        ktab[tid] = ch < Ci ? sh[smp * Ci + ch] : 0.f;
    }
    __syncthreads();
    f32x16_t acc[9];
#pragma unroll
    for (int t = 0; t < 9; t++)
#pragma unroll
        for (int r = 0; r < 16; r++) acc[t][r] = 0.f;

    constexpr int CG = GP / 16, CX = XP / 16, PPG = 1024 / GP, PPX = 1024 / XP;
    constexpr int PG = C::NGP / NW, PX = (C::NXP + NW - 1) / NW;
    static_assert(C::NGP % NW == 0 && PG + PX == C::PW, "piece split");
    const int cg = lane % CG, pg = lane / CG, cx = lane % CX, px = lane / CX;
    const bool g_alive = o0 + cg * 8 < Co, x_alive = i0 + cx * 8 < Ci;
    const bool last_x = wave + NW * (PX - 1) < C::NXP;
    const int pw_mine = PG + PX - (last_x ? 0 : 1);
    unsigned rel_g[PG], rel_x[PX];
#pragma unroll
    for (int j = 0; j < PG; j++) {
        const int q = (wave + NW * j) * PPG + pg;
        rel_g[j] = g_alive ? (unsigned)((((q >> 4) * W + (q & 15)) * Co + o0 + cg * 8) * 2) : DEAD;
    }
#pragma unroll
    for (int j = 0; j < PX; j++) {
        const int q = (wave + NW * j) * PPX + px, hy = q / C::HWD, hx = q - hy * C::HWD;
        rel_x[j] = (q < C::HH * C::HWD && x_alive) ? (unsigned)((((hy - 1) * W + (hx - 1)) * Ci + i0 + cx * 8) * 2) : DEAD;
    }
    const unsigned lds0 = lds_off(lds);
    const unsigned sample_g = (unsigned)H * W * Co * 2, sample_x = (unsigned)H * W * Ci * 2;
    int irem = t_begin - smp * tps, ity = irem / tiles_x, itx = irem - ity * tiles_x;
    auto issue = [&](int stage) {
        const unsigned mg = lds0 + stage * C::STAGE + wave * 1024, mx = mg + C::GBYTES;
        const int y0 = ity * TH, x0 = itx * 16;
        const rsrc_t rg = make_rsrc((unsigned long long)g + (unsigned long long)smp * sample_g, sample_g);
        const rsrc_t rx = make_rsrc((unsigned long long)X + (unsigned long long)smp * sample_x, sample_x);
        const unsigned gbase = (unsigned)((y0 * W + x0) * Co * 2), xbase = (unsigned)((y0 * W + x0) * Ci * 2);
        const bool interior = (y0 >= 1) & (y0 + TH + 1 <= H) & (x0 >= 1) & (x0 + 17 <= W);
        if (interior) {
#pragma unroll
            for (int j = 0; j < PG; j++) dma16(gbase + rel_g[j], rg, mg + j * NW * 1024);
#pragma unroll
            for (int j = 0; j < PX - 1; j++) dma16(xbase + rel_x[j], rx, mx + j * NW * 1024);
            if (last_x) dma16(xbase + rel_x[PX - 1], rx, mx + (PX - 1) * NW * 1024);
        } else {
#pragma unroll
            for (int j = 0; j < PG; j++) {
                const int q = (wave + NW * j) * PPG + pg;
                const bool ok = (rel_g[j] != DEAD) & (y0 + (q >> 4) < H) & (x0 + (q & 15) < W);
                dma16(ok ? gbase + rel_g[j] : DEAD, rg, mg + j * NW * 1024);
            }
#pragma unroll
            for (int j = 0; j < PX; j++) {
                const int q = (wave + NW * j) * PPX + px, hy = q / C::HWD, hx = q - hy * C::HWD;
                const bool ok = (rel_x[j] != DEAD) & ((unsigned)(y0 + hy - 1) < (unsigned)H) & ((unsigned)(x0 + hx - 1) < (unsigned)W);
                if (j < PX - 1 || last_x) dma16(ok ? xbase + rel_x[j] : DEAD, rx, mx + j * NW * 1024);
            }
        }
        if (++itx == tiles_x) { itx = 0; ++ity; }
    };
    auto wait_tile = [&](int nfly) {
        const bool full = pw_mine == C::PW;
#define DGE_W(N) asm volatile("s_waitcnt vmcnt(%0)" :: "i"(N) : "memory")
        if (nfly <= 0) DGE_W(0);
        else if (nfly == 1) { if (full) DGE_W(C::PW); else DGE_W(C::PW - 1); }
// ... 14 lines not shown
        float v[9] = {s_tot, s_top, s_bot, s_lft, s_rgt, s_tl, s_tr, s_bl, s_br};
        float* part = (float*)lds;
        __syncthreads();
#pragma unroll
        for (int k = 0; k < 9; k++) {
            v[k] += __shfl_xor(v[k], 32, 64);
            if (lane < 32) part[(wave * 9 + k) * 32 + lane] = v[k];
        }
        __syncthreads();
        for (int idx = tid; idx < 9 * 32; idx += NT) {
            float t = 0.f;
#pragma unroll
            for (int w = 0; w < NW; w++) t += part[w * 9 * 32 + idx];
            gtab[idx] = t;
        }
        __syncthreads();
    };

#pragma unroll
    for (int s = 0; s < NS - 1; s++) if (t_begin + s < t_end) issue(s);
    int stage = 0;
#ifdef DGE_WG_TIMING
    const bool tlogon = lin == 40 && tid == 0;
#endif
    for (int t = t_begin; t < t_end; t++) {
        const int younger = t_end - 1 - t;
        DGE_WT(0);
        wait_tile(younger < NS - 2 ? younger : NS - 2);
        DGE_WT(1);
        __syncthreads();
        DGE_WT(2);
        if (t + NS - 1 < t_end) issue(stage == 0 ? NS - 1 : stage - 1);
        DGE_WT(3);
        const unsigned char* sg = lds + stage * C::STAGE;
        const unsigned char* sx = sg + C::GBYTES;
        const int y0 = cty * TH, x0 = ctx * 16;
        const bool edge_tile = (y0 == 0) | (y0 + TH >= H) | (x0 == 0) | (x0 + 16 >= W);
        uint4 av[2];
        uint4 xv[2][3];
        uint32_t xw[2][3];
        auto frags = [&](int rr, uint4& a, uint4 (&x3)[3], uint32_t (&w3)[3]) {
            const int row = C::RW * wave + rr;
            const unsigned char* ga = sg + row * 16 * GP + frag_g;
            const v4s_t a0 = trd(ga), a1 = trd(ga + 4 * GP);
            const uint2 a01 = *(const uint2*)&a0, a23 = *(const uint2*)&a1;
            a = make_uint4(a01.x, a01.y, a23.x, a23.y);
#pragma unroll
            for (int dy = 0; dy < 3; dy++) {
                const unsigned char* xa = sx + (row + dy) * C::HWD * XP + frag_x;
                const v4s_t q0 = trd(xa), q1 = trd(xa + 4 * XP), q2 = trd(xa + 8 * XP);
                const uint2 w01 = *(const uint2*)&q0, w23 = *(const uint2*)&q1;
                x3[dy] = make_uint4(w01.x, w01.y, w23.x, w23.y);
                w3[dy] = (*(const uint2*)&q2).x;
            }
        };
        frags(0, av[0], xv[0], xw[0]);
        StaticFor<C::RW>::run([&](auto rc) {
            constexpr int rr = decltype(rc)::value;
            if constexpr (rr + 1 < C::RW) frags(rr + 1, av[(rr + 1) & 1], xv[(rr + 1) & 1], xw[(rr + 1) & 1]);
            const uint4 a4 = av[rr & 1];
            const bf16x8_t a = *(const bf16x8_t*)&a4;
#pragma unroll
            for (int dy = 0; dy < 3; dy++) {
                const uint4 v0 = xv[rr & 1][dy];
                const uint32_t w4 = xw[rr & 1][dy];
                const uint4 b1 = make_uint4(__builtin_amdgcn_alignbit(v0.y, v0.x, 16), __builtin_amdgcn_alignbit(v0.z, v0.y, 16),
                                            __builtin_amdgcn_alignbit(v0.w, v0.z, 16), __builtin_amdgcn_alignbit(w4, v0.w, 16));
                const uint4 b2 = make_uint4(v0.y, v0.z, v0.w, w4);
// ... 65 lines not shown
            stg[(ol * 32 + il) * 9 + t] = s;
        }
    }
    __syncthreads();
    if (dots) {
        red[tid * 2] = d_s2; red[tid * 2 + 1] = d_s1;
        __syncthreads();
        if (tid < 64) {
            const int il = tid & 31, k = tid >> 5;
            float v = 0.f;
            for (int j = 0; j < NT / 32; j++) v += red[(il + 32 * j) * 2 + k];
            if (i0 + il < Ci) atomicAdd(dots + ((size_t)(grp_id % dots_slots) * B * Ci + (size_t)smp * Ci + i0 + il) * 2 + k, v);
        }
    }
    const int ni = (Ci - i0 < 32 ? Ci - i0 : 32) * 9;
    if (det_on()) {
        const int L = 1024 * 9, nslots = B * gps;
        float* dslot = det_slot(oi, noi, grp_id, nslots, L);
        for (int idx = tid; idx < L; idx += NT) dslot[idx] = stg[idx];
        if (det_arrive_wg(oi, nslots)) {
            for (int idx = tid; idx < L; idx += NT) {
                const int ol = idx / (32 * 9), j = idx - ol * (32 * 9);
                if (o0 + ol < Co && j < ni) dW[((size_t)(o0 + ol) * Ci + i0) * 9 + j] += det_sum(oi, nslots, L, idx);
            }
        }
        return;
    }
    for (int idx = tid; idx < 1024 * 9; idx += NT) {
        const int ol = idx / (32 * 9), j = idx - ol * (32 * 9);
        if (o0 + ol < Co && j < ni) atomicAdd(dW + ((size_t)(o0 + ol) * Ci + i0) * 9 + j, stg[idx]);
    }
}

template <class C>
int launch(const void* g, const void* x, const float* sc, const float* sh, float* dw, int B, int H, int W, int cout, int cin,
           const float* wdot, float* dots, int dots_slots, hipStream_t s) {
    const int tx = (W + 15) / 16, ty = (H + C::TH - 1) / C::TH;
    const int tps = tx * ty;
    const int noi = ((cout + 31) / 32) * ((cin + 31) / 32);
    const int lds_bytes = C::lds_bytes();
    static int attr_bytes[16] = {0};
    int dev = 0;
    (void)hipGetDevice(&dev);
    auto kern = wgrad_dma_kernel<C>;
    if (dev < 0 || dev >= 16 || attr_bytes[dev] < lds_bytes) {
        const hipError_t e = hipFuncSetAttribute((const void*)kern, hipFuncAttributeMaxDynamicSharedMemorySize, lds_bytes);
        if (e != hipSuccess) {
            dge_set_error("wgrad_dma: cannot raise the dynamic LDS limit to %d bytes: %s", lds_bytes, hipGetErrorString(e));
            return -3;
        }
        if (dev >= 0 && dev < 16) attr_bytes[dev] = lds_bytes;
    }
    const int wg_per_cu = 2 * lds_bytes <= 160 * 1024 ? 2 : 1;
    const int groups_env = dge_env().wgrad_groups;
    int gps = groups_env > 0 ? groups_env : (256 * wg_per_cu + noi * B - 1) / (noi * B);
    gps = gps < 1 ? 1 : (gps > tps ? tps : gps);
    const int per = (tps + gps - 1) / gps;
    gps = (tps + per - 1) / per;
    const int groups = B * gps;
    const int groups8 = groups < 8 ? groups : (groups + 7) / 8 * 8;
    if (!dge_det_fits(noi, (long long)B * gps, 1024 * 9)) return 1;
    dge_note_kernel("wgrad_dma<%d,%d,%d,%d>", C::TH, C::GP, C::XP, C::NS);
    hipLaunchKernelGGL(kern, dim3(noi, groups8), dim3(C::NW * 64), lds_bytes, s, (const bf16_t*)g, (const bf16_t*)x, sc, sh, dw, B, H, W,
                       cout, cin, tx, ty, per, gps, wdot, dots, dots_slots < 1 ? 1 : dots_slots);
    DGE_LAUNCH_CHECK("wgrad_dma");
    return 0;
}

}

#ifdef DGE_WG_TIMING
extern "C" int dge_wgrad_tlog(long long* out, int n) {
    return (int)hipMemcpyFromSymbol(out, HIP_SYMBOL(wg_tlog), (size_t)n * sizeof(long long), 0, hipMemcpyDeviceToHost);
}
#endif
int dge_wgrad_dma_try(const void* g, const void* x, const float* sc, const float* sh, float* dw, int B, int H, int W, int cout, int cin,
                      const float* wdot, float* dots, int dots_slots, hipStream_t s) {
    static int off = -1;
    if (off < 0) off = getenv("DGE_NO_WGRAD_DMA") ? 1 : 0;
    if (off) return 1;
    if (cout % 8 || cin % 8) return 1;
    if (dots && (!sc || !wdot || !dge_det_fits(1LL << 40, 1, 1))) return 1;
    if ((size_t)H * W * cout * 2 >= (1u << 30) || (size_t)H * W * cin * 2 >= (1u << 30)) return 1;
    const int tps = ((W + 15) / 16) * ((H + 15) / 16);
    const int noi = ((cout + 31) / 32) * ((cin + 31) / 32);
    if (tps < 16 || noi * B > 1024) return 1;
    const bool g32 = cout <= 16, x32 = cin <= 16;
    {
        static const int cfg = getenv("DGE_WGRAD_CFG") ? atoi(getenv("DGE_WGRAD_CFG")) : 0;
#define WTRY(...) return launch<WCfg<__VA_ARGS__>>(g, x, sc, sh, dw, B, H, W, cout, cin, wdot, dots, dots_slots, s)
        if (cfg == 1) { if (g32 && x32) WTRY(8, 32, 32, 4, 5); if (!g32 && x32) WTRY(8, 64, 32, 4, 4); if (!g32 && !x32) WTRY(8, 64, 64, 4, 4); }
        if (cfg == 2) { if (g32 && x32) WTRY(16, 32, 32, 4, 4); if (!g32 && x32) WTRY(16, 64, 32, 4, 3); if (!g32 && !x32) WTRY(16, 64, 64, 4, 3); }
        if (cfg == 3) { if (g32 && x32) WTRY(8, 32, 32, 4, 3); if (!g32 && x32) WTRY(8, 64, 32, 4, 3); if (!g32 && !x32) WTRY(8, 64, 64, 4, 3); }
#undef WTRY
    }
    if (g32 && x32) return launch<WCfg<16, 32, 32, 4, 3>>(g, x, sc, sh, dw, B, H, W, cout, cin, wdot, dots, dots_slots, s);
    if (!g32 && x32) return launch<WCfg<16, 64, 32, 4, 2>>(g, x, sc, sh, dw, B, H, W, cout, cin, wdot, dots, dots_slots, s);
    if (g32 && !x32) return launch<WCfg<16, 32, 64, 4, 2>>(g, x, sc, sh, dw, B, H, W, cout, cin, wdot, dots, dots_slots, s);
    if (cin <= 32 && cout <= 64) return launch<WCfg<8, 64, 64, 4, 3>>(g, x, sc, sh, dw, B, H, W, cout, cin, wdot, dots, dots_slots, s);
    return launch<WCfg<16, 64, 64, 4, 2>>(g, x, sc, sh, dw, B, H, W, cout, cin, wdot, dots, dots_slots, s);
}
```

### deep-gan-encoders_amd/ops.py

```python
import ctypes as C
import math

import torch

from ._lib import lib, check, ConvDesc, ConvPPDesc, DgeError, last_kernel

F32, BF16 = 0, 1
ACT_NONE, ACT_LRELU, ACT_RELU, LIN_RSQRT = 0, 1, 2, 3
PACK_FWD, PACK_UPFOLD, PACK_DGRAD, PACK_UPFOLD_DGRAD, PACK_SG1_UP, PACK_SG1_UP_DGRAD, PACK_UPT2D_DGRAD = 0, 1, 2, 3, 4, 5, 6
PACK_FRAG = 0x100
import os as _os
import weakref as _weakref
_PF = {"on": not _os.environ.get("DGE_NO_PREFETCH"), "prev": {}, "next": {}}
KERNEL_LOG = None
PROFILE = None


class _ZeroArena:

    def __init__(self):
        self.buf, self.off, self.high, self.active = None, 0, 0, False


_ARENA = _ZeroArena()
# ... 273 lines not shown
    if not x.is_cuda or x.stride(1) != 1:
        raise DgeError("dense_chain: x must be a CUDA tensor with unit inner stride")
    check(lib().dge_dense_chain(_f32(x), x.stride(0), arr, len(layers), _p(y), y.stride(0), B, 1 if pixelnorm else 0, float(eps), _stream()),
          "dge_dense_chain")
    return y


def pixelnorm(x, eps=1e-8):
    y = torch.empty_like(x)
    check(lib().dge_pixelnorm(_f32(x), _p(y), x.shape[0], x.shape[1], eps, _stream()), "dge_pixelnorm")
    return y


def truncation(w, w_avg, num_layers, psi, layers):
    w_is_wp = (w.ndim == 3)
    B, D = w.shape[0], w.shape[-1]
    wp = torch.empty((B, num_layers, D), dtype=torch.float32, device=w.device)
    check(lib().dge_truncation(_f32(w.contiguous()), _f32(w_avg), _p(wp), B, num_layers, D, float(psi), int(layers),
                               1 if w_is_wp else 0, _stream()), "dge_truncation")
    return wp


def conv2d(x, w_packed, cout, ksize=3, up=False, in_scale=None, in_shift=None, out_scale=None, bias=None,
           bias_scale=1.0, noise=None, noise_w=None, act=ACT_NONE, gain=1.0, addend=None, add_scale=1.0, stats=None,
           out=None, in_s2d=False, dot_src=None, in_up2=False, in_relu=False, prep=None, relu_mask=None, in_t2d=False, rgb=None, pool_out=False, pool_mask=False,
           in_bwd=None):
    B, H, W, Cin = x.shape
    if in_s2d:
        H, W, Cin = H // 2, W // 2, Cin * 4
    if in_up2:
        H, W = 2 * H, 2 * W
    if in_t2d:
        H, W = H - 1, W - 1
    dt = dtype_of(x)
    OH, OW = (2 * H, 2 * W) if up else (H, W)
    mask = None
    if pool_out:
        if out is not None or up:
            raise DgeError("conv2d: pool_out allocates its own result and excludes up")
        out = torch.empty((B, OH // 2, OW // 2, cout), dtype=x.dtype, device=x.device)
        if pool_mask:
            mask = torch.empty((B, (OH // 2) * (OW // 2), cout // 8), dtype=torch.int32, device=x.device)
    if out is None:
        out = torch.empty((B, OH, OW, cout), dtype=x.dtype, device=x.device)
    d = ConvDesc()
    d.pool_out, d.pool_mask = 1 if pool_out else 0, _p(mask)
    if relu_mask is not None:
        if dot_src is not None or prep is not None:
            raise DgeError("conv2d: relu_mask excludes dot_src / prep")
        dot_src = relu_mask
    d.mask_relu = 0 if relu_mask is None else 1
    d.in_t2d = 1 if in_t2d else 0
    d.x, d.w_packed, d.y, d.addend, d.dot_src = _p(x), _p(w_packed), _p(out), _p(addend), _p(dot_src)
    d.in_scale, d.in_shift, d.out_scale = _f32(in_scale), _f32(in_shift), _f32(out_scale)
    partial, nslot = None, 1
    lazy = isinstance(stats, SlotStats)
    if stats is not None:
        nblk = ((H + 15) // 16) * ((W + 15) // 16) * B
        nslot = max(1, min(64, nblk // 16))
        if lazy:
            partial = stats.alloc(nslot)
        elif nslot > 1:
            partial = zeros((nslot,) + tuple(stats.shape), x.device)
    d.bias, d.noise, d.noise_w, d.stats = _f32(bias), _f32(noise), _f32(noise_w), _f32(partial if partial is not None else stats)
    d.stats_slots = nslot
    d.B, d.H, d.W, d.Cin, d.Cout = B, H, W, Cin, cout
# ... 3 lines not shown
    if d.w_layout and _PF["on"]:
        sk = (_stream().value or 0)
        key = w_packed.data_ptr()
        prev = _PF["prev"].get(sk) if isinstance(_PF["prev"], dict) else None
        if not isinstance(_PF["prev"], dict):
            _PF["prev"] = {}
        if prev is not None and prev != key:
            if len(_PF["next"]) > 512:
                _PF["next"].clear()
            _PF["next"][(sk, prev)] = (key, w_packed.shape[1], w_packed.shape[2], _weakref.ref(w_packed))
        _PF["prev"][sk] = key
        nxt = _PF["next"].get((sk, key))
        if nxt is not None:
            t = nxt[3]()
            if t is None or t.data_ptr() != nxt[0]:
                del _PF["next"][(sk, key)]
            else:
                d.prefetch_w, d.prefetch_ntot, d.prefetch_cin = C.c_void_p(nxt[0]), int(nxt[1]), int(nxt[2])
    if prep is not None:
        if stats is None or dot_src is None:
            raise DgeError("conv2d: prep needs stats and dot_src")
        pn = prep.get("noise")
        d.prep, d.prep_gain = 1, float(prep["gain"])
        d.prep_noise, d.prep_ns = _f32(pn), _f32(prep.get("ns") if pn is not None else None)
        d.prep_noise_batch = 1 if pn is None else pn.shape[0]
        d.prep_stats = _f32(prep["stats"].alloc(nslot))
    if in_bwd is not None:
        if dot_src is None or stats is not None or prep is not None:
            raise DgeError("conv2d: in_bwd needs dot_src and excludes stats / prep")
        nblk = ((H + 15) // 16) * ((W + 15) // 16) * B
        d.stats_slots = max(1, min(64, nblk // 16))
        pn = in_bwd.get("noise")
        d.in_bwd_coef = _f32(in_bwd["coef"])
        d.prep_noise, d.prep_noise_batch = _f32(pn), 1 if pn is None else pn.shape[0]
        if in_bwd.get("fr") is not None:
            d.fr_img4, d.in_bwd_extra, d.in_bwd_extra_scale = _f32(in_bwd["img4"]), _p(in_bwd.get("extra")), float(in_bwd.get("extra_scale", 1.0))
            in_bwd["fr"].buf = zeros((d.stats_slots, B, cout, 4), x.device)
            d.fr_out = _f32(in_bwd["fr"].buf)
        elif in_bwd.get("red") is not None:
            d.prep_stats = _f32(in_bwd["red"].alloc(d.stats_slots))
        else:
            d.prep_noise = None
            d.in_bwd_extra, d.in_bwd_extra_scale = _p(in_bwd.get("extra")), float(in_bwd.get("extra_scale", 1.0))
    if rgb is not None:
        d.rgb_w, d.rgb_style, d.rgb_bias, d.rgb_out = _f32(rgb["w"]), _f32(rgb["style"]), _f32(rgb["bias"]), _f32(rgb["out"])
        d.rgb_wscale, d.rgb_skip_y = float(rgb["wscale"]), 1 if rgb.get("skip_y") else 0
    d.noise_batch = 1 if noise is None else noise.shape[0]
    d.noise_w_per_channel = 0 if (noise_w is None or noise_w.numel() == 1) else 1
    d.act, d.bias_scale, d.gain, d.add_scale, d.dtype = act, bias_scale, gain, add_scale, dt
    if w_packed.dtype != x.dtype:
        raise DgeError("conv2d: packed weight dtype differs from activation dtype")
    if PROFILE is not None:
        e0, e1 = torch.cuda.Event(enable_timing=True), torch.cuda.Event(enable_timing=True)
        e0.record()
        check(lib().dge_conv2d(C.byref(d), _stream()), "dge_conv2d")
        e1.record()
        if up:
            macs = 9.0 * Cin * cout * H * W
        elif in_s2d or in_t2d:
            macs = 9.0 * (Cin // 4) * cout * H * W
        else:
            macs = float(ksize * ksize) * Cin * cout * H * W
        skip_y = rgb is not None and rgb.get("skip_y")
        abytes = sum(t.numel() * t.element_size() for t in (x, None if skip_y else out, addend, dot_src, w_packed,
                                                            rgb["out"] if rgb is not None else None) if t is not None)
        PROFILE.append((e0, e1, 2.0 * macs * B, (B, H, W, Cin, cout, ksize, up, in_s2d), abytes))
    else:
        check(lib().dge_conv2d(C.byref(d), _stream()), "dge_conv2d")
    if partial is not None and not lazy:
        check(lib().dge_sum_slots(_p(partial), _p(stats), nslot, stats.numel(), 1, _stream()), "dge_sum_slots")
    if rgb is not None and rgb.get("skip_y"):
        return None
    if pool_out and pool_mask:
        return out, mask
    return out


def conv_in_bwd_supported(B, H, W, cin, cout, dtype):
    return bool(lib().dge_conv_in_bwd_supported(int(B), int(H), int(W), int(cin), int(cout), 3, int(dtype)))


def conv_in_bwd_x_supported(B, H, W, cin, cout, dtype):
    return bool(lib().dge_conv_in_bwd_x_supported(int(B), int(H), int(W), int(cin), int(cout), 3, int(dtype)))


def conv_in_bwd_fromrgb_supported(B, H, W, cin, cout, dtype):
    return bool(lib().dge_conv_in_bwd_fromrgb_supported(int(B), int(H), int(W), int(cin), int(cout), 3, int(dtype)))


def up_pp_supported(B, H, W, cin, cout, dtype):
    return bool(lib().dge_up_pp_supported(int(B), int(H), int(W), int(cin), int(cout), int(dtype)))


def pack_up_pp(w_units, cout, cin, in_scale=None, out_scale=None, gain=1.0, out=None):
    if w_units.dtype != torch.bfloat16:
        raise DgeError("pack_up_pp: expects the bf16 units of pack_upconv_weight")
    nb = 1
    for t in (in_scale, out_scale):
        if t is not None:
            nb = t.shape[0]
    if out is None:
        out = torch.empty((nb, 9 * cin * cout), dtype=torch.bfloat16, device=w_units.device)
    check(lib().dge_pack_up_pp(_p(w_units), _p(out), int(cout), int(cin), _f32(in_scale), _f32(out_scale), float(gain), nb, _stream()),
          "dge_pack_up_pp")
    return out


def up_pp(x, w_img, cout, bias=None, bias_scale=1.0, noise=None, noise_w=None, act=ACT_NONE, gain=1.0):
    B, H, W, Cin = x.shape
    if x.dtype != torch.bfloat16 or not x.is_cuda:
        raise DgeError("up_pp: bf16 CUDA activations only (the HIP path has no CPU fallback)")
    y = torch.empty((B, 2 * H, 2 * W, cout), dtype=x.dtype, device=x.device)
# ... 260 lines not shown


def up2_bwd(g):
    B, Cc, H, W = g.shape
    out = torch.empty((B, Cc, H // 2, W // 2), dtype=torch.float32, device=g.device)
    check(lib().dge_up2_bwd(_f32(g), _p(out), B * Cc, H // 2, W // 2, _stream()), "dge_up2_bwd")
    return out


def conv_wgrad(g, x, dw, in_scale=None, in_shift=None):
    B, H, W, Cin = x.shape
    cout, _, k, _ = dw.shape
    check(lib().dge_conv_wgrad(_p(g), _p(x), _f32(in_scale), _f32(in_shift), _f32(dw), B, H, W, cout, Cin, k, dtype_of(x),
                               _stream()), "dge_conv_wgrad")
    return dw


def conv_wgrad_dots(g, x, dw, in_scale, in_shift, w, dots):
    B, H, W, Cin = x.shape
    cout = dw.shape[0]
    if dw.shape[2] != 3 or is_deterministic():
        return False
    nslot = max(1, min(16, (H * W) // 4096))
    buf = dots.alloc(nslot)
    r = lib().dge_conv_wgrad_dots(_p(g), _p(x), _f32(in_scale), _f32(in_shift), _f32(dw), _f32(w.detach()), _f32(buf), nslot, B, H, W, cout, Cin,
                                  dtype_of(x), _stream())
    if r == 1:
        dots.buf, dots.nslot = None, 1
        return False
    check(r, "dge_conv_wgrad_dots")
    return True


class DeferredSums:

    def __init__(self):
        self.items = []

    def add(self, part, red):
        self.items.append((part, red))
        if len(self.items) == 32:
            self.flush()
        return red

    def flush(self):
        if not self.items:
            return
        from ._lib import SumPlanarEntry
        arr = (SumPlanarEntry * len(self.items))()
        for e, (part, red) in zip(arr, self.items):
            e.partial, e.out = _p(part), _p(red)
            e.nslot, e.C, e.NS = part.shape
        check(lib().dge_sum_slots_planar_multi(arr, len(self.items), _stream()), "dge_sum_slots_planar_multi")
        self.items = []


def _sum_planar(part, red, defer=None):
    if defer is not None:
        return defer.add(part, red)
    B, Cc, NS = part.shape
    check(lib().dge_sum_slots_planar(_p(part), _p(red), B, Cc, NS, _stream()), "dge_sum_slots_planar")
    return red


def act_bwd(gup, a, noise=None, pool=False, scale=1.0, red=None, slope=0.2, planar=False, defer=None):
    B, H, W, Cc = a.shape
    gpre = torch.empty_like(a)
    ncol = 2 if red is None else (red.shape[0] if planar else red.shape[-1])
    part = zeros((B, Cc, ncol), a.device) if red is not None else None
    check(lib().dge_act_bwd(_p(gup), _p(a), _f32(noise), _p(gpre), _f32(part), ncol, B, H, W, Cc,
                            1 if pool else 0, float(scale), float(slope), dtype_of(a), _stream()), "dge_act_bwd")
    if red is not None:
        _sum_planar(part, red, defer) if planar else _sum_over_batch(part, red)
    return gpre


def act_bwd_mask(gup, mask, noise, scale=1.0, red=None, slope=0.2, planar=False, defer=None):
    B, UH, UW, Cc = gup.shape
    H, W = 2 * UH, 2 * UW
    gpre = torch.empty((B, H, W, Cc), dtype=gup.dtype, device=gup.device)
    ncol = 2 if red is None else (red.shape[0] if planar else red.shape[-1])
    part = zeros((B, Cc, ncol), gup.device) if red is not None else None
    check(lib().dge_act_bwd_mask(_p(gup), _p(mask), _f32(noise), _p(gpre), _f32(part), ncol, B, H, W, Cc, float(scale), float(slope),
                                 dtype_of(gup), _stream()), "dge_act_bwd_mask")
    if red is not None:
        _sum_planar(part, red, defer) if planar else _sum_over_batch(part, red)
    return gpre


def in_bwd_coef(dots, gms, musig, sc, sh, npix):
    B, Cc = sc.shape
    coef = torch.empty((B, Cc, 3), dtype=torch.float32, device=sc.device)
    nslot = 1
    if isinstance(dots, SlotStats):
        nslot, dots = dots.nslot, dots.buf
    check(lib().dge_in_bwd_coef_slots(_f32(dots), nslot, _f32(gms), _f32(musig), _f32(sc), _f32(sh), _p(coef), B, Cc, int(npix),
                                      _stream()), "dge_in_bwd_coef")
    return coef


def in_bwd(gy, x, coef, extra=None, extra_pool=False, extra_scale=1.0, noise=None, act=False, red=None, planar=False, defer=None):
    B, H, W, Cc = x.shape
    gout = torch.empty_like(x)
    part = zeros((B, Cc, 2), x.device) if red is not None else None
    if isinstance(coef, tuple) and Cc > 512:
        coef = in_bwd_coef(*coef)
    if isinstance(coef, tuple):
        dots, gms, musig, sc, sh, npix = coef
        nslot = 1
        if isinstance(dots, SlotStats):
            nslot, dots = dots.nslot, dots.buf
        check(lib().dge_in_bwd_fused(_p(gy), _p(x), _f32(dots), nslot, _f32(gms), _f32(musig), _f32(sc), _f32(sh), int(npix), _p(extra),
                                     _f32(noise), _p(gout), _f32(part), B, H, W, Cc, 1 if extra_pool else 0, float(extra_scale),
# ... 327 lines not shown
```

### include/dge_hip.h

```cpp
#ifndef DGE_HIP_H
#define DGE_HIP_H
#include <stddef.h>
#ifdef __cplusplus
extern "C" {
#endif

typedef struct ihipStream_t* dge_stream_t;

#define DGE_DTYPE_F32 0
#define DGE_DTYPE_BF16 1
#define DGE_ACT_LINEAR 0
#define DGE_ACT_LRELU02 1
#define DGE_ACT_RELU_ 2
#define DGE_LIN_RSQRT 3
#define DGE_PACK_FWD 0
#define DGE_PACK_UPFOLD 1
#define DGE_PACK_DGRAD 2
#define DGE_PACK_UPFOLD_DGRAD 3
#define DGE_PACK_SG1_UP 4
#define DGE_PACK_SG1_UP_DGRAD 5
#define DGE_PACK_UPT2D_DGRAD 6

const char* dge_last_error(void);
int dge_version(void);
// ... 17 lines not shown
    int in_s2d;
    int noise_batch;
    int noise_w_per_channel;
    int act;
    float bias_scale, gain, add_scale;
    int dtype;
    int in_up2;
    int in_relu;
    int stats_slots;
    int w_layout;
    int prep;
    float prep_gain;
    const float* prep_noise;
    const float* prep_ns;
    int prep_noise_batch;
    float* prep_stats;
    int mask_relu;
    int in_t2d;
    const float* rgb_w;
    const float* rgb_style;
    const float* rgb_bias;
    float* rgb_out;
    float rgb_wscale;
    int rgb_skip_y;
    int pool_out;
    void* pool_mask;
    const void* prefetch_w;
    int prefetch_ntot, prefetch_cin;
    const float* in_bwd_coef;
    const void* in_bwd_extra;
    float in_bwd_extra_scale;
    const float* fr_img4;
    float* fr_out;
} dge_conv_desc;
int dge_conv2d(const dge_conv_desc* d, dge_stream_t stream);
int dge_conv_small_supported(int H, int W, int cin, int ntot, int ksize, int in_s2d, int in_up2, int dtype);
#define DGE_PACK_FRAG 0x100
const char* dge_last_kernel(void);
void dge_env_reload(void);
int dge_sum_slots(const float* partial, float* out, int nslot, int n, int accumulate, dge_stream_t stream);
int dge_sum_slots_planar(const float* partial, float* out, int nslot, int C, int NS, dge_stream_t stream);
typedef struct dge_sum_planar_entry { const float* partial; float* out; int nslot, C, NS, pad; } dge_sum_planar_entry;
int dge_sum_slots_planar_multi(const dge_sum_planar_entry* entries, int n, dge_stream_t stream);

int dge_linear_rows(const float* x, int ldx_b, const int* row_xoff, const float* w, const float* bias, float* y,
                    const int* row_ybase, const int* row_ybstride, int B, int R, int K, float wscale, float bscale, float add,
                    dge_stream_t stream);
int dge_demod_rows(const float* s_all, const float* wsq_cat, const int* row_woff, const int* row_sbase, const int* row_cin,
                   float* d_all, const int* row_dbase, const int* row_dbstride, int B, int R, float eps, dge_stream_t stream);
int dge_set_deterministic(int on);
int dge_get_deterministic(void);
int dge_packed_n(int n_valid);
int dge_pack_conv_weight(const float* w_oihw, void* out, int cout, int cin, int ksize, int mode, int dtype,
                         float scale, dge_stream_t stream);
int dge_pack_conv_weights_multi(const long long* table_host, void* descs_dev, int n, int upload, dge_stream_t stream);
int dge_pack_desc_bytes(void);
int dge_weight_sumsq(const float* w_oihw, float* wsq, int cout, int cin, int ksize, float scale, dge_stream_t stream);

int dge_linear(const float* x, int ldx, const float* w, const float* bias, float* y, int ldy, int B, int I, int O,
               float wscale, float bscale, float add, int act, float gain, int square_input, dge_stream_t stream);
int dge_pixelnorm(const float* x, float* y, int B, int D, float eps, dge_stream_t stream);
typedef struct dge_dense_layer { const float* w; const float* bias; int I, O; float wscale, bscale, add; int act; float gain; } dge_dense_layer;
int dge_dense_chain(const float* x, int ldx, const dge_dense_layer* layers, int n, float* y, int ldy, int B, int pixelnorm, float eps,
                    dge_stream_t stream);
int dge_truncation(const float* w, const float* w_avg, float* wp, int B, int L, int D, float psi, int layers,
                   int w_is_wp, dge_stream_t stream);

int dge_torgb(const void* x, const float* wrgb, const float* style, const float* bias, const float* prev, float* img,
              int B, int H, int W, int cin, float wscale, int dtype, dge_stream_t stream);

int dge_conv_rgb_supported(int B, int H, int W, int Cin, int Cout, int ksize, int dtype);
int dge_conv_in_bwd_supported(int B, int H, int W, int Cin, int Cout, int ksize, int dtype);
int dge_conv_in_bwd_fromrgb_supported(int B, int H, int W, int Cin, int Cout, int ksize, int dtype);
int dge_conv_in_bwd_x_supported(int B, int H, int W, int Cin, int Cout, int ksize, int dtype);
int dge_conv_pool_supported(int B, int H, int W, int Cin, int Cout, int ksize, int dtype);
int dge_rgb_upsample_add(float* img, const float* prev, int BC, int H, int W, dge_stream_t stream);
int dge_nchw_to_nhwc(const float* src, void* dst, int B, int C, int HW, int src_B, int dtype, dge_stream_t stream);
int dge_nhwc_to_nchw(const void* src, float* dst, int B, int C, int HW, int dtype, dge_stream_t stream);

int dge_fromrgb(const float* img, const float* w, const float* bias, void* y, float* stats, int B, int HW, int C,
                int dtype, dge_stream_t stream);
int dge_fromrgb2(const float* img, const float* w, const float* bias, void* y, float* stats, float* img4, int B, int HW, int C,
                 int dtype, dge_stream_t stream);
int dge_stats_finalize(const float* stats, float* musig, float* sc, float* sh, int B, int C, int npix, float eps,
                       dge_stream_t stream);
int dge_stats_finalize_slots(const float* stats, int nslot, float* musig, float* sc, float* sh, int B, int C, int npix, float eps,
                             dge_stream_t stream);
int dge_blend(const void* x, const void* z, void* y, const float* sc, const float* sh, float* stats, int B, int OH,
              int OW, int C, int pool, float alpha, float beta, int dtype, dge_stream_t stream);

int dge_loss_reduce(const float* a, const float* b, float* sums7, int B, int C, int H, int W, int y0, int x0, int h, int w,
                    dge_stream_t stream);
int dge_crop_pool(const float* src, float* dst, int BC, int H, int W, int y0, int x0, int h, int w, int k, dge_stream_t stream);
int dge_ssim_fwd(const float* a, const float* b, float* ssim_sum, float* dmap, int BC, int h, int w, dge_stream_t stream);
int dge_ssim_box7(const float* a, const float* b, float* sums, int BC, int h, int w, float scale, float shift, float data_range,
                  dge_stream_t stream);
int dge_ssim_bwd(const float* a, const float* b, const float* dmap, float* g, int BC, int h, int w, float scale,
                 int accumulate, dge_stream_t stream);
int dge_space_loss_finalize(const float* sums7, const float* ssim_sum, const float* lpips, float* out8, float n,
                            float n_pooled, int image_space, dge_stream_t stream);
int dge_space_loss_bwd(const float* a, const float* b, const float* sums7, const float* g_pooled, float* g, int BC, int H,
                       int W, int y0, int x0, int h, int w, int k, float n, float weight, int accumulate, dge_stream_t stream);
int dge_loss_reduce3(const float* a, const float* b, float* sums, int B, int C, int H, int W, const int* wins, int nwin, dge_stream_t stream);
int dge_crop_pool_multi(const float* const* src, float* const* dst, const int* wins, const int* ks, int n, int BC, int H, int W,
                        dge_stream_t stream);
int dge_space_loss_bwd3(const float* a, const float* b, const float* const* sums7, const float* const* g_pooled, float* g, int BC, int H,
                        int W, const int* wins, const int* ks, const float* n, const float* weight, int nwin, dge_stream_t stream);
// ... 9 lines not shown
int dge_modconv_bwd_prep(const void* gx, const void* x, const float* d, const float* noise, void* gy, float* R, int B,
                         int HW, int C, int noise_batch, float gain, int dtype, dge_stream_t stream);
int dge_demod_bwd(const float* R, const float* d, const float* bias, const float* noise_strength, float* t, int B, int C,
                  float bscale, dge_stream_t stream);
int dge_linear_t(const float* x, int ldx, int incx, const float* w, const float* mul, float* y, int ldy, int incy, int B,
                 int O, int K, float scale, int accumulate, dge_stream_t stream);
int dge_torgb_bwd(const float* gimg, const void* x, const float* wrgb, const float* style, void* gx, float* gs, int B,
                  int HW, int C, float wscale, int dtype, dge_stream_t stream);
int dge_torgb_bwd_prep(const float* gimg, const void* x, const float* wrgb, const float* style, const float* noise,
                       const float* noise_strength, int noise_batch, void* gz, float* gs, float* P, int B, int HW, int C,
                       float wscale, float gain, int dtype, dge_stream_t stream);
int dge_fir_t2d(const void* g, const float* scale, void* z, int B, int H, int W, int C, int dtype, dge_stream_t stream);
typedef struct dge_s2_grad_entry {
    const float* P; const float* st; const float* d; const float* s; const float* bias; const float* wsq;
    const float* gs; const float* wstyle;
    int nslot_p, nslot_s, in_c, out_c, row;
    float bscale;
} dge_s2_grad_entry;
int dge_s2_style_grads(const dge_s2_grad_entry* entries, int n, float* g_wp, int B, int nrows, int K, float wscale, dge_stream_t stream);
int dge_demod_bwd_prep(const float* P, int nslot, const float* d, const float* bias, float* t, int B, int C, float bscale,
                       dge_stream_t stream);
int dge_up2_bwd(const float* g, float* gprev, int BC, int h, int w, dge_stream_t stream);

int dge_conv_wgrad(const void* g, const void* x, const float* in_scale, const float* in_shift, float* dw, int B, int H, int W,
                   int cout, int cin, int ksize, int dtype, dge_stream_t stream);
int dge_conv_wgrad_dots(const void* g, const void* x, const float* in_scale, const float* in_shift, float* dw, const float* w,
                        float* dots, int dots_slots, int B, int H, int W, int cout, int cin, int dtype, dge_stream_t stream);
int dge_act_bwd(const void* gup, const void* a, const float* noise, void* gpre, float* red, int red_cols, int B, int H, int W, int C,
                int pool, float scale, float slope, int dtype, dge_stream_t stream);
int dge_blend_pool_mask(const void* x, const void* z, void* y, float* stats, unsigned* mask, int B, int OH, int OW, int C, float alpha,
                        float beta, int dtype, dge_stream_t stream);
int dge_act_bwd_mask(const void* gup, const unsigned* mask, const float* noise, void* gpre, float* red, int red_cols, int B, int H, int W,
                     int C, float scale, float slope, int dtype, dge_stream_t stream);
int dge_fromrgb_dgrad(const void* gx, const void* x0, const float* w, float* gimg, int B, int HW, int C, int dtype, dge_stream_t stream);
int dge_nearest_up2(const void* x, void* y, int B, int H, int W, int C, float scale, int dtype, dge_stream_t stream);
int dge_in_bwd_coef(const float* dots, const float* gms, const float* musig, const float* sc, const float* sh, float* coef,
                    int B, int C, int npix, dge_stream_t stream);
int dge_in_bwd_coef_slots(const float* dots, int nslot, const float* gms, const float* musig, const float* sc, const float* sh,
                          float* coef, int B, int C, int npix, dge_stream_t stream);
int dge_in_bwd(const void* gy, const void* x, const float* coef, const void* extra, const float* noise, void* gout, float* red,
               int B, int H, int W, int C, int extra_pool, float extra_scale, int act, int dtype, dge_stream_t stream);
int dge_in_bwd_fused(const void* gy, const void* x, const float* dots, int nslot, const float* gms, const float* musig,
                     const float* sc, const float* sh, int npix, const void* extra, const float* noise, void* gout, float* red,
                     int B, int H, int W, int C, int extra_pool, float extra_scale, int act, int dtype, dge_stream_t stream);
int dge_chan_sum(const void* x, float* out, int B, int HW, int C, float scale, int dtype, dge_stream_t stream);
int dge_fromrgb_bwd(const void* gx, const void* x0, const float* img, float* out4, int B, int HW, int C, int dtype,
                    dge_stream_t stream);
int dge_in_bwd_fromrgb(const void* gy, const void* x0, const float* dots, int nslot, const float* gms, const float* musig,
                       const float* sc, const float* sh, int npix, const void* extra, const float* img, float* out4,
                       int B, int H, int W, int C, int extra_pool, float extra_scale, int dtype, dge_stream_t stream);
int dge_heads_fwd(const void* dev_entries, int n, const float* musig_all, float* w, int ldw, int B, int O, dge_stream_t stream);
int dge_head_entry_size(void);
int dge_heads_bwd(const void* dev_entries, int n, int max_I, const float* g, int ldg, const float* musig_all, float* gms_all,
                  float* gw_all, float* gb_all, int B, int O, dge_stream_t stream);
int dge_dense_wgrad(const float* gy, int ldgy, const float* x, int ldx, float* gw, float* gb, int B, int O, int I,
                    int accumulate, dge_stream_t stream);

int dge_lpips_prep(const float* img, void* x, int B, int HW, int cpad, const float* host_shift3, const float* host_scale3,
                   int dtype, dge_stream_t stream);
int dge_lpips_prep_bwd(const void* gx, float* gimg, int B, int HW, int cpad, const float* host_scale3, float factor,
                       int accumulate, int dtype, dge_stream_t stream);
int dge_maxpool2(const void* x, void* y, int B, int H, int W, int C, int dtype, dge_stream_t stream);
int dge_maxpool2_bwd(const void* gy, const void* x, const void* addend, void* gx, int B, int H, int W, int C, int dtype,
                     dge_stream_t stream);
int dge_lpips_head(const void* feat, const float* lin, float* val, void* g1, int B, int HW, int C, float gscale, int dtype,
                   dge_stream_t stream);
// ... 117 lines not shown
```

Baseline: 358.4 images/sec.

## Expand pooled activation gradient inside wgrad and dgrad conv kernels instead of materializing

Instead of writing the full-resolution pre-activation gradient g_pre2 (upsampled pooled gradient times leaky-ReLU mask) to memory, the encoder backward now passes the pooled gradient and bitmask directly. The weight-gradient kernel and the streaming data-gradient conv each expand it on the fly in LDS. This removes a full-resolution bf16 write and two reads for the large early encoder blocks. In exchange it adds expansion work and LDS staging inside both kernels, and a more constrained slot and vmcnt plan.

```diff
diff --git a/deep-gan-encoders_amd/_lib.py b/deep-gan-encoders_amd/_lib.py
--- a/deep-gan-encoders_amd/_lib.py
+++ b/deep-gan-encoders_amd/_lib.py
@@ -24,6 +24,7 @@
         ("rgb_skip_y", C.c_int), ("pool_out", C.c_int), ("pool_mask", C.c_void_p),
         ("prefetch_w", C.c_void_p), ("prefetch_ntot", C.c_int), ("prefetch_cin", C.c_int), ("in_bwd_coef", C.c_void_p),
         ("in_bwd_extra", C.c_void_p), ("in_bwd_extra_scale", C.c_float), ("fr_img4", C.c_void_p), ("fr_out", C.c_void_p),
+        ("pg_mask", C.c_void_p), ("pg_scale", C.c_float), ("pg_slope", C.c_float),
     ]
 
 
@@ -77,6 +78,7 @@
     "dge_torgb": [_P, _P, _P, _P, _P, _P, _I, _I, _I, _I, _F, _I, _P],
     "dge_conv_rgb_supported": [_I, _I, _I, _I, _I, _I, _I],
     "dge_conv_in_bwd_supported": [_I, _I, _I, _I, _I, _I, _I],
+    "dge_conv_pooled_g_supported": [_I, _I, _I, _I, _I, _I, _I],
     "dge_conv_in_bwd_fromrgb_supported": [_I, _I, _I, _I, _I, _I, _I],
     "dge_conv_in_bwd_x_supported": [_I, _I, _I, _I, _I, _I, _I],
     "dge_conv_pool_supported": [_I, _I, _I, _I, _I, _I, _I],
@@ -174,6 +176,7 @@
     "dge_pack_conv_pp": [_P, _P, _I, _I, _F, _P, _P, _F, _I, _I, _P],
     "dge_dense_chain": [_P, _I, C.POINTER(DenseLayer), _I, _P, _I, _I, _I, _F, _P],
     "dge_conv_wgrad_dots": [_P, _P, _P, _P, _P, _P, _P, _I, _I, _I, _I, _I, _I, _I, _P],
+    "dge_conv_wgrad_dots_pooled": [_P, _P, _F, _F, _P, _P, _P, _P, _P, _P, _I, _I, _I, _I, _I, _I, _I, _P],
     "dge_pack_conv_pp_rows": [_P, _I, _P, _I, _I, _P, _I, _P, _F, _I, _I, _P],
     "dge_conv_pp": [C.POINTER(ConvPPDesc), _P],
     "dge_up_pp_supported": [_I, _I, _I, _I, _I, _I],
diff --git a/deep-gan-encoders_amd/autograd_enc_bwd.py b/deep-gan-encoders_amd/autograd_enc_bwd.py
--- a/deep-gan-encoders_amd/autograd_enc_bwd.py
+++ b/deep-gan-encoders_amd/autograd_enc_bwd.py
@@ -7,6 +7,7 @@
 from .weight_cache import pack_cache, packed
 
 FUSE_IN_BWD = not os.environ.get("DGE_NO_FUSED_IN_BWD")
+POOLED_GPRE = os.environ.get("DGE_POOLED_GPRE", "1") != "0"
 
 
 def encoder_backward(E, saved, g_w):
@@ -67,13 +68,23 @@
             if g_out is None:
                 raise RuntimeError("non-final encoder block without an output gradient")
             red2 = ops.zeros((3 if has3 else 2, C2), dev)
-            g_pre2 = ops.act_bwd_mask(g_out, rec["m2"], rec["n2"], scale=0.111 * 0.25, red=red2, planar=True, defer=later)
+            pooled2 = None
+            if POOLED_GPRE and FUSE_IN_BWD and ops.conv_in_bwd_supported(B, H, H, C2, Cc, dt) and ops.conv_pooled_g_supported(B, H, H, C2, Cc, dt):
+                pooled2 = dict(mask=rec["m2"], scale=0.111 * 0.25, slope=0.2)
+            g_pre2 = ops.act_bwd_mask(g_out, rec["m2"], rec["n2"], scale=0.111 * 0.25, red=red2, planar=True, defer=later,
+                                      store=pooled2 is None)
             grads[pre + "bias_2"] = red2[0].reshape(1, C2, 1, 1)
             grads[pre + "noise_weight_2"] = red2[1].reshape(1, C2, 1, 1)
             gW2 = ops.zeros(tuple(blk.conv_2.weight.shape), dev)
             dots2 = ops.SlotStats(B, Cc, dev)
-            fuse2 = FUSE_IN_BWD and ops.conv_in_bwd_supported(B, H, H, C2, Cc, dt) and \
-                ops.conv_wgrad_dots(g_pre2, x1, gW2, rec["sc2"], rec["sh2"], blk.conv_2.weight, dots2)
+            if pooled2 is not None:
+                fuse2 = ops.conv_wgrad_dots_pooled(g_out, pooled2["mask"], pooled2["scale"], x1, gW2, rec["sc2"], rec["sh2"],
+                                                   blk.conv_2.weight, dots2, slope=pooled2["slope"])
+                if not fuse2:
+                    raise RuntimeError("conv_pooled_g_supported() accepted a shape the pooled weight gradient does not cover")
+            else:
+                fuse2 = FUSE_IN_BWD and ops.conv_in_bwd_supported(B, H, H, C2, Cc, dt) and \
+                    ops.conv_wgrad_dots(g_pre2, x1, gW2, rec["sc2"], rec["sh2"], blk.conv_2.weight, dots2)
             if not fuse2:
                 ops.conv_wgrad(g_pre2, x1, gW2, rec["sc2"], rec["sh2"])
             grads[pre + "conv_2.weight"] = gW2
@@ -96,8 +107,8 @@
         red1 = ops.zeros((2, Cc), dev)
         if fuse2:
             redp = ops.SlotStats(B, Cc, dev)
-            g_pre1 = ops.conv2d(g_pre2, packed(cache, blk.conv_2, dt, ops.PACK_DGRAD, H), Cc, 3, dot_src=x1,
-                                in_bwd=dict(coef=ops.in_bwd_coef(*coef2), noise=rec["n1"].reshape(B, H, H), red=redp))
+            g_pre1 = ops.conv2d(g_out if pooled2 is not None else g_pre2, packed(cache, blk.conv_2, dt, ops.PACK_DGRAD, H), Cc, 3, dot_src=x1,
+                                in_bwd=dict(coef=ops.in_bwd_coef(*coef2), noise=rec["n1"].reshape(B, H, H), red=redp, pooled=pooled2))
             ops._sum_planar(redp.buf.view(-1, Cc, 2), red1, later)
         else:
             g_pre1 = ops.in_bwd(g_y2, x1, coef2, noise=rec["n1"], act=True, red=red1, planar=True, defer=later)
diff --git a/deep-gan-encoders_amd/csrc/capi.hip b/deep-gan-encoders_amd/csrc/capi.hip
--- a/deep-gan-encoders_amd/csrc/capi.hip
+++ b/deep-gan-encoders_amd/csrc/capi.hip
@@ -118,6 +118,8 @@
     p.in_coef = d->in_bwd_coef;
     p.in_extra = d->in_bwd_coef ? d->in_bwd_extra : nullptr; p.in_extra_scale = d->in_bwd_extra_scale;
     p.fr_img4 = d->in_bwd_coef ? d->fr_img4 : nullptr; p.fr_out = d->in_bwd_coef ? d->fr_out : nullptr;
+    p.pg_mask = (const unsigned*)d->pg_mask; p.pg_scale = d->pg_scale; p.pg_slope = d->pg_slope;
+    DGE_CHECK(!d->pg_mask || (d->in_bwd_coef && d->prep_stats && !d->fr_out), "conv2d: pg_mask goes with in_bwd_coef and prep_stats");
     if (d->in_bwd_coef) {
         DGE_CHECK(!dge_get_deterministic(), "conv2d: in_bwd_coef is not offered in deterministic mode; run dge_in_bwd");
         DGE_CHECK(d->ksize == 3 && !d->up && dge_conv_stream_eligible(p, d->dtype, d->ksize), "conv2d: in_bwd_coef is offered where "
@@ -146,6 +148,14 @@
     p.B = B; p.H = H; p.W = W; p.Cin = Cin; p.Cout = Cout; p.Ntot_valid = Cout; p.Ntot = dge_packed_n(Cout);
     p.dot_src = (const void*)16; p.prep_stats = (float*)16; p.in_coef = (const float*)16;
     return (ksize == 3 && !dge_get_deterministic() && dge_conv_stream_eligible(p, dtype, ksize)) ? 1 : 0;
+}
+bool dge_wgrad_dma_pooled_ok(int B, int H, int W, int cout, int cin);
+extern "C" int dge_conv_pooled_g_supported(int B, int H, int W, int Cin, int Cout, int ksize, int dtype) {
+    ConvParams p = {};
+    p.B = B; p.H = H; p.W = W; p.Cin = Cin; p.Cout = Cout; p.Ntot_valid = Cout; p.Ntot = dge_packed_n(Cout);
+    p.dot_src = (const void*)16; p.prep_stats = (float*)16; p.in_coef = (const float*)16; p.pg_mask = (const unsigned*)16;
+    return (ksize == 3 && dtype == DGE_BF16 && !dge_get_deterministic() && dge_conv_stream_eligible(p, dtype, ksize) &&
+            dge_wgrad_dma_pooled_ok(B, H, W, Cin, Cout)) ? 1 : 0;
 }
 extern "C" int dge_conv_in_bwd_x_supported(int B, int H, int W, int Cin, int Cout, int ksize, int dtype) {
     ConvParams p = {};
diff --git a/deep-gan-encoders_amd/csrc/conv_params.h b/deep-gan-encoders_amd/csrc/conv_params.h
--- a/deep-gan-encoders_amd/csrc/conv_params.h
+++ b/deep-gan-encoders_amd/csrc/conv_params.h
@@ -49,6 +49,7 @@
     int pf_ntot, pf_cin;
     const float* in_coef;
     const void* in_extra; float in_extra_scale; const float* fr_img4; float* fr_out;
+    const unsigned* pg_mask; float pg_scale, pg_slope;
 };
 
 int dge_conv_launch(const ConvParams& p, int dtype, int ksize, hipStream_t s);
diff --git a/deep-gan-encoders_amd/csrc/conv_stream.hip b/deep-gan-encoders_amd/csrc/conv_stream.hip
--- a/deep-gan-encoders_amd/csrc/conv_stream.hip
+++ b/deep-gan-encoders_amd/csrc/conv_stream.hip
@@ -65,7 +65,7 @@
                      "buffer_load_dwordx4 %3, %2, 0 offen offset:1024 lds" : : "v"(voff), "s"(m0v), "s"(rs), "v"(voff1) : "memory");
 }
 
-enum { FL_GEN = 0, FL_ENC = 1, FL_ENC_STATS = 2, FL_DOT = 3, FL_DOT_PREP = 4, FL_GEN_RGB = 5, FL_ENC_POOL = 6, FL_DOT_IN = 7, FL_DOT_FR = 8, FL_DOT_INX = 9 };
+enum { FL_GEN = 0, FL_ENC = 1, FL_ENC_STATS = 2, FL_DOT = 3, FL_DOT_PREP = 4, FL_GEN_RGB = 5, FL_ENC_POOL = 6, FL_DOT_IN = 7, FL_DOT_FR = 8, FL_DOT_INX = 9, FL_DOT_INP = 10 };
 
 template <int CIN, int COUT, int FL>
 struct SC {
@@ -76,7 +76,7 @@
     static constexpr int MTW = MT / TEAM;
     static constexpr int HW = 34, RB = HW * PXB;
     static constexpr int PIECES = (RB + 1023) / 1024;
-    static constexpr bool PREP = FL == FL_DOT_PREP, RGB = FL == FL_GEN_RGB, POOL = FL == FL_ENC_POOL, FRB = FL == FL_DOT_FR, INX = FL == FL_DOT_INX, INB = FL == FL_DOT_IN || FRB || INX;
+    static constexpr bool PREP = FL == FL_DOT_PREP, RGB = FL == FL_GEN_RGB, POOL = FL == FL_ENC_POOL, FRB = FL == FL_DOT_FR, INX = FL == FL_DOT_INX, PGI = FL == FL_DOT_INP, INB = FL == FL_DOT_IN || FRB || INX || PGI;
     static_assert(!RGB || COUT == 32 || (COUT == 64 && TEAM == 2), "fused toRGB: 32 output channels per wave, one wave or a 2-wave team per pixel");
     static constexpr bool DOT = FL == FL_DOT || PREP || INB, STATS = FL == FL_ENC_STATS, ENC = FL == FL_ENC || FL == FL_ENC_STATS || POOL;
     static constexpr bool NOISE = !DOT || PREP || (INB && !FRB && !INX);
@@ -92,7 +92,9 @@
     static constexpr int DROWB = 32 * DCH * 16, DPIECES = DROWB / 1024;
     static_assert(!DOT || MTW == 1, "data-gradient mode: one M tile per wave");
     static constexpr int XPW = TEAM == 2 ? (PIECES + 1) / 2 : PIECES;
-    static constexpr int LPR = XPW + (DOT ? DPIECES : 0) + (FRB ? 2 : 0) + (INX ? 1 : 0);
+    static constexpr int PG_MOFF = 18 * PXB, PGP = (PG_MOFF + 1023) / 1024, PGL = PGI ? PGP + 1 : 0;
+    static_assert(!PGI || (TEAM == 1 && PG_MOFF + 1024 <= RB && (CIN == 32 || CIN == 64)), "pooled-gradient input: staged inside one ring row");
+    static constexpr int LPR = (PGI ? 0 : XPW) + (DOT ? DPIECES : 0) + (FRB ? 2 : 0) + (INX ? 1 : 0);
     static constexpr int X_OFF = 0;
     static constexpr int XRING = NR * RB;
     static constexpr int N_OFF = (XRING + 1023) / 1024 * 1024;
@@ -112,7 +114,8 @@
     static constexpr int NEED = 4 * 9 * KS * MTW + 32 * MTW + 16 + (ENC ? 16 * MTW : 0) + (STATS || DOT ? 32 * MTW : 0) + (DOT ? 16 : 0) + (PREP ? 16 : 0) + (RGB ? 11 : 0) + (POOL ? 20 * MTW : 0) + 36;
     static constexpr int WPE = ((PREP || INB) && CIN == 64) ? 1 : (NEED <= 128 ? 4 : (NEED <= 168 ? 3 : 2));
     static_assert(D <= NR - 3, "the slot of the row being fetched must be dead");
-    static_assert((D - 1) * LPR + 1 < 64, "vmcnt range");
+    static_assert((D - 1) * LPR + 1 + PGL < 64, "vmcnt range");
+    static_assert(!PGI || (D == 2 && NR == 6), "pooled-gradient input: the slot plan below");
 };
 
 template <int LOGC> __device__ __forceinline__ int chunk_swz(int px) { return (px >> (4 - LOGC)) & ((1 << LOGC) - 1); }
@@ -189,11 +192,13 @@
     unsigned long long dptr = DOTb + (unsigned long long)(long long)(r0 - 2) * yrow_bytes;
     auto issue = [&](int h, int slot, int slot_d) {
         const int gy = r0 - 1 + h;
-        const bool xv = (unsigned)gy < (unsigned)p.H && h <= rows + 1;
-        const rsrc_t rx = make_rsrc(xptr, xv ? xrow_bytes : 0u);
-        xptr += xrow_bytes;
-        const unsigned m0x = lds0 + C::X_OFF + slot * C::RB;
-        dma_row<CIN, C::TEAM>(wave, voff, voff_b, voff_c, rx, rs_null, m0x, lds0 + C::DUMMY_OFF);
+        if constexpr (!C::PGI) {
+            const bool xv = (unsigned)gy < (unsigned)p.H && h <= rows + 1;
+            const rsrc_t rx = make_rsrc(xptr, xv ? xrow_bytes : 0u);
+            xptr += xrow_bytes;
+            const unsigned m0x = lds0 + C::X_OFF + slot * C::RB;
+            dma_row<CIN, C::TEAM>(wave, voff, voff_b, voff_c, rx, rs_null, m0x, lds0 + C::DUMMY_OFF);
+        }
         const bool ov = h >= 2 && h <= rows + 1;
         if constexpr (C::DOT) {
             const rsrc_t rd = make_rsrc(dptr, ov ? yrow_bytes : 0u);
@@ -221,8 +226,71 @@
         const rsrc_t rn = make_rsrc(NZb + (unsigned long long)(v ? gy : 0) * nzrow_bytes, v ? (unsigned)(p.H - gy) * nzrow_bytes : 0u);
         dma_piece(nvoff, rn, lds0 + C::N_OFF + wave * C::NRING + buf_off);
     };
+    const unsigned pgrow_bytes = C::PGI ? (unsigned)(p.W >> 1) * C::PXB : 0u, pgmrow_bytes = C::PGI ? (unsigned)(p.W >> 1) * C::CH * 4u : 0u;
+    const unsigned long long PGb = C::PGI ? (unsigned long long)p.x + (unsigned long long)b * (p.H >> 1) * pgrow_bytes : Xb;
+    const unsigned long long PGMb = C::PGI ? (unsigned long long)p.pg_mask + (unsigned long long)b * (p.H >> 1) * pgmrow_bytes : Xb;
+    const unsigned pg_voff = (unsigned)(((x0 >> 1) - 1) * C::PXB + lane * 16), pgm_voff = (unsigned)(((x0 >> 1) - 1) * C::CH * 4 + lane * 16);
+    const float pg_scale = C::PGI ? p.pg_scale : 1.f, pg_slope = C::PGI ? p.pg_slope : 1.f;
+    auto issue_pg = [&](int q, int slot) {
+        const int pr = (r0 >> 1) - 1 + q;
+        const bool v = (unsigned)pr < (unsigned)(p.H >> 1);
+        const rsrc_t rg = make_rsrc(PGb + (unsigned long long)(v ? pr : 0) * pgrow_bytes, v ? pgrow_bytes : 0u);
+        const rsrc_t rm = make_rsrc(PGMb + (unsigned long long)(v ? pr : 0) * pgmrow_bytes, v ? pgmrow_bytes : 0u);
+        const unsigned m0g = lds0 + C::X_OFF + slot * C::RB;
+        unsigned long long keep;
+        if constexpr (CIN == 32)
+            asm volatile(DGE_M0 DGE_P(0) DGE_MASK(0xff) DGE_P(1024) DGE_UNMASK : "=&s"(keep) : "v"(pg_voff), "s"(m0g), "s"(rg) : "memory");
+        else
+            asm volatile(DGE_M0 DGE_P(0) DGE_P(1024) DGE_MASK(0xffff) DGE_P(2048) DGE_UNMASK : "=&s"(keep) : "v"(pg_voff), "s"(m0g), "s"(rg) : "memory");
+        dma_piece(pgm_voff, rm, m0g + C::PG_MOFF);
+    };
+    typedef unsigned u32x4w_t __attribute__((ext_vector_type(4)));
+    typedef __attribute__((address_space(3))) u32x4w_t* lds_w4p;
+    unsigned lds0v = 0;
+    if constexpr (C::PGI) asm("v_mov_b32 %0, %1" : "=v"(lds0v) : "s"(lds0));
+    auto expand_pg = [&](int src, int up, int dn) {
+        const unsigned sb = lds0v + C::X_OFF + src * C::RB;
+        constexpr int PPR = 64 / C::CH, NRND = 16 / PPR;
+        const int c = lane & (C::CH - 1);
+        const bool edge = lane < 2 * C::CH;
+        const int je = lane < C::CH ? 0 : 17;
+        u32x4w_t gv[NRND + 1]; unsigned mv[NRND + 1];
+#pragma unroll
+        for (int r = 0; r <= NRND; r++) {
+            const int j = r < NRND ? 1 + r * PPR + (lane >> C::LOGCH) : je;
+            if (r < NRND || edge) {
+                gv[r] = *(const lds_w4p)(sb + (unsigned)((j * C::CH + c) * 16));
+                mv[r] = *(const __attribute__((address_space(3))) unsigned*)(sb + (unsigned)(C::PG_MOFF + (j * C::CH + c) * 4));
+            }
+        }
+#pragma unroll
+        for (int r = 0; r <= NRND; r++) {
+            const int j = r < NRND ? 1 + r * PPR + (lane >> C::LOGCH) : je;
+            if (r < NRND || edge) {
+                float f[8];
+                unpack16(make_uint4(gv[r][0], gv[r][1], gv[r][2], gv[r][3]), f, (bf16_t*)nullptr);
+#pragma unroll
+                for (int e = 0; e < 8; e++) f[e] *= pg_scale;
+#pragma unroll
+                for (int k = 0; k < (r < NRND ? 4 : 2); k++) {
+                    const int dy = r < NRND ? k >> 1 : k, dx = r < NRND ? k & 1 : (je == 0 ? 1 : 0), c4 = 2 * dy + dx;
+                    if (dy == 0 && up < 0) continue;
+                    const unsigned bits = mv[r] >> (c4 * 8);
+                    float o[8];
+#pragma unroll
+                    for (int e = 0; e < 8; e++) o[e] = f[e] * (((bits >> e) & 1u) ? 1.f : pg_slope);
+                    const uint4 ov = pack16(o, (bf16_t*)nullptr);
+                    const int hp = 2 * j - 1 + dx;
+                    const unsigned a = lds0v + C::X_OFF + (unsigned)((dy ? dn : up) * C::RB + hp * C::PXB + ((c ^ chunk_swz<C::LOGCH>(hp)) << 4));
+                    u32x4w_t w4; w4[0] = ov.x; w4[1] = ov.y; w4[2] = ov.z; w4[3] = ov.w;
+                    *(lds_w4p)a = w4;
+                }
+            }
+        }
+    };
     asm volatile("s_waitcnt vmcnt(0)" ::: "memory");
     if constexpr (C::NOISE) issue_noise(0, 0u);
+    if constexpr (C::PGI) { issue_pg(0, 4); issue_pg(1, 5); issue_pg(2, 3); }
     StaticFor<C::D + 2>::run([&](auto hc) { constexpr int h = decltype(hc)::value; issue(h, h % C::NR, (h + C::NR - 2) % C::NR % C::DR); });
 
     uint4 wf[C::MTW][9][C::KS];
@@ -409,13 +477,18 @@
     auto step = [&](auto ic, int s, unsigned npar) {
         constexpr int I = decltype(ic)::value;
         DGE_T(0);
-        constexpr int NAFTER = (C::D - 1) * C::LPR + ((C::NOISE && I >= 1 && I <= C::D - 1) ? 1 : 0);
+        constexpr int NAFTER = (C::D - 1) * C::LPR + ((C::NOISE && I >= 1 && I <= C::D - 1) ? 1 : 0) + ((C::PGI && (I & 1)) ? C::PGL : 0);
         asm volatile("s_waitcnt vmcnt(%0)" :: "i"(NAFTER) : "memory");
         if constexpr (C::RGB && C::TEAM == 2) asm volatile("s_waitcnt lgkmcnt(0)" ::: "memory");
         if constexpr (C::TEAM == 2) __builtin_amdgcn_s_barrier();
         if constexpr (C::RGB && C::TEAM == 2) { if (wave == 0 && s > 0) rgb_flush(s - 1); }
         DGE_T(1);
         if constexpr (C::NOISE && I == 0) issue_noise(s + C::NR, npar ^ 1024u);
+        if constexpr (C::PGI && (I & 1) == 0) {
+            issue_pg((s >> 1) + 3, (I + 5) % C::NR);
+            expand_pg((I + 3) % C::NR, (I + 3) % C::NR, (I + 4) % C::NR);
+            __builtin_amdgcn_sched_barrier(0);
+        }
         issue(s + 2 + C::D, (I + 2 + C::D) % C::NR, (I + C::D) % C::DR);
         DGE_T(2);
 
@@ -612,6 +685,12 @@
     const long long tj1 = __builtin_readcyclecounter();
     __builtin_amdgcn_sched_barrier(0);
 #endif
+    if constexpr (C::PGI) {
+        asm volatile("s_waitcnt vmcnt(%0)" :: "i"(C::PGL + (C::D + 2) * C::DPIECES) : "memory");
+        expand_pg(4, -1, 0);
+        expand_pg(5, 1, 2);
+        __builtin_amdgcn_sched_barrier(0);
+    }
     unsigned npar = 0;
     for (int s0_ = 0; s0_ < rows; s0_ += C::NR, npar ^= 1024u) {
         bool done = false;
@@ -715,12 +794,12 @@
     if (nseg > maxseg) nseg = maxseg;
     if (nseg < 1) nseg = 1;
     int seg_rows = (p.H + nseg - 1) / nseg;
-    if (C::POOL) seg_rows += seg_rows & 1;
+    if (C::POOL || C::PGI) seg_rows += seg_rows & 1;
     nseg = (p.H + seg_rows - 1) / seg_rows;
     const int njobs = p.B * nstrips * nseg;
     const int nwg = (njobs + C::TPW - 1) / C::TPW;
     const int jobs_per_xcd = (nwg + 7) / 8;
-    const char* fl = FL == FL_GEN ? "gen" : (FL == FL_ENC ? "enc" : (FL == FL_ENC_STATS ? "enc_stats" : (FL == FL_DOT ? "dot" : (FL == FL_DOT_PREP ? "dot_prep" : (FL == FL_GEN_RGB ? "gen_rgb" : (FL == FL_DOT_IN ? "dot_in" : (FL == FL_DOT_FR ? "dot_fromrgb" : (FL == FL_DOT_INX ? "dot_inx" : "enc_pool"))))))));
+    const char* fl = FL == FL_GEN ? "gen" : (FL == FL_ENC ? "enc" : (FL == FL_ENC_STATS ? "enc_stats" : (FL == FL_DOT ? "dot" : (FL == FL_DOT_PREP ? "dot_prep" : (FL == FL_GEN_RGB ? "gen_rgb" : ((FL == FL_DOT_IN || FL == FL_DOT_INP) ? "dot_in" : (FL == FL_DOT_FR ? "dot_fromrgb" : (FL == FL_DOT_INX ? "dot_inx" : "enc_pool"))))))));
     dge_note_kernel("conv_stream<bf16,%d,%d,%s>", CIN, COUT, fl);
     hipLaunchKernelGGL(kern, dim3((unsigned)(jobs_per_xcd * 8)), dim3(64 * C::TEAM * C::TPW), C::LDS_BYTES * C::TPW, s, p, nstrips, nseg, seg_rows, njobs, jobs_per_xcd);
     DGE_LAUNCH_CHECK("conv_stream");
@@ -740,7 +819,10 @@
         return -1;
     }
     if (p.in_coef) {
-        if constexpr ((CIN == 32 && COUT == 16) || (CIN == 64 && COUT == 32)) return launch_stream<CIN, COUT, FL_DOT_IN>(p, s);
+        if constexpr ((CIN == 32 && COUT == 16) || (CIN == 64 && COUT == 32)) {
+            if (p.pg_mask) return launch_stream<CIN, COUT, FL_DOT_INP>(p, s);
+            return launch_stream<CIN, COUT, FL_DOT_IN>(p, s);
+        }
         dge_set_error("conv_stream: the instance-norm backward epilogue is built for 32 -> 16 and 64 -> 32 only");
         return -1;
     }
@@ -795,6 +877,7 @@
     if (p.Cin == 64 && !p.dot_src && (p.stats || p.in_shift || (p.noise && p.noise_w_stride != 0))) return false;
     if (p.dot_src && (p.bias || p.noise || p.in_shift || p.act != DGE_ACT_NONE)) return false;
     if (p.noise && p.noise_w == nullptr) return false;
+    if (p.pg_mask && !(p.in_coef && !p.fr_out && p.prep_stats && p.H % 2 == 0 && p.W % 2 == 0)) return false;
     if (dge_env().no_stream) return false;
     return true;
 }
diff --git a/deep-gan-encoders_amd/csrc/enc_bwd_kernels.hip b/deep-gan-encoders_amd/csrc/enc_bwd_kernels.hip
--- a/deep-gan-encoders_amd/csrc/enc_bwd_kernels.hip
+++ b/deep-gan-encoders_amd/csrc/enc_bwd_kernels.hip
@@ -345,7 +345,7 @@
     if (red_out) block_chan_flush<EP, NS>(s, cpt, ppi, red_out + (size_t)b * C * NS, C, red);
 }
 
-template <typename T, int NS>
+template <typename T, int NS, bool STORE = true>
 __global__ __launch_bounds__(256) void act_bwd_mask_kernel(const T* __restrict__ gup, const unsigned* __restrict__ mask,
                                                             const float* __restrict__ noise, T* __restrict__ gpre,
                                                             float* __restrict__ red_out, int H, int W, int C, float scale, float slope) {
@@ -399,7 +399,7 @@
                     o[e] = g[e] * (((m >> (c4 * EP + e)) & 1u) ? 1.f : slope);
                     s[0][e] += o[e]; s[1][e] += o[e] * nz;
                 }
-                *(uint4*)(gpre + ((size_t)b * HW + p) * C + chunk * EP) = pack16(o, (T*)nullptr);
+                if constexpr (STORE) *(uint4*)(gpre + ((size_t)b * HW + p) * C + chunk * EP) = pack16(o, (T*)nullptr);
             }
         }
     }
@@ -706,6 +706,15 @@
     if (dtype != DGE_BF16) return 1;
     return dge_wgrad_dma_try(g, x, in_scale, in_shift, dw, B, H, W, cout, cin, w, dots, dots_slots, s);
 }
+int dge_wgrad_dma_pooled_try(const void* gup, const unsigned* mask, float scale, float slope, const void* x, const float* sc, const float* sh,
+                             float* dw, int B, int H, int W, int cout, int cin, const float* wdot, float* dots, int dots_slots, hipStream_t s);
+extern "C" int dge_conv_wgrad_dots_pooled(const void* gup, const unsigned* mask, float scale, float slope, const void* x, const float* in_scale,
+                                          const float* in_shift, float* dw, const float* w, float* dots, int dots_slots, int B, int H, int W,
+                                          int cout, int cin, int dtype, hipStream_t s) {
+    DGE_CHECK(gup && mask && x && dw && w && dots && in_scale && in_shift && dots_slots >= 1, "conv_wgrad_dots_pooled: null tensor");
+    if (dtype != DGE_BF16) return 1;
+    return dge_wgrad_dma_pooled_try(gup, mask, scale, slope, x, in_scale, in_shift, dw, B, H, W, cout, cin, w, dots, dots_slots, s);
+}
 extern "C" int dge_conv_wgrad(const void* g, const void* x, const float* in_scale, const float* in_shift, float* dw, int B, int H,
                               int W, int cout, int cin, int ksize, int dtype, hipStream_t s) {
     DGE_CHECK(ksize == 1 || ksize == 3, "conv_wgrad: ksize %d unsupported", ksize);
@@ -789,8 +798,10 @@
     const int ep = dtype == DGE_BF16 ? 8 : 4;
     DGE_CHECK(CHAN_OK(C, ep) && H % 2 == 0 && W % 2 == 0 && mask, "act_bwd_mask: unsupported shape (C %d, %d x %d)", C, H, W);
     DGE_CHECK(red_cols == 2 || red_cols == 3, "act_bwd_mask: red_cols must be 2 or 3 (got %d)", red_cols);
+    DGE_CHECK(gpre || red, "act_bwd_mask: neither a result nor reductions wanted");
     dim3 grid(dge_stream_grid(H * W / 4, 256 / (C / ep), B), B);
-#define AB(T, NS) hipLaunchKernelGGL((act_bwd_mask_kernel<T, NS>), grid, dim3(256), 0, s, (const T*)gup, mask, noise, (T*)gpre, red, H, W, C, scale, slope)
+#define AB(T, NS) do { if (gpre) hipLaunchKernelGGL((act_bwd_mask_kernel<T, NS, true>), grid, dim3(256), 0, s, (const T*)gup, mask, noise, (T*)gpre, red, H, W, C, scale, slope); \
+                       else hipLaunchKernelGGL((act_bwd_mask_kernel<T, NS, false>), grid, dim3(256), 0, s, (const T*)gup, mask, noise, (T*)nullptr, red, H, W, C, scale, slope); } while (0)
     if (dtype == DGE_BF16) { if (red_cols == 3) AB(bf16_t, 3); else AB(bf16_t, 2); }
     else { if (red_cols == 3) AB(float, 3); else AB(float, 2); }
 #undef AB
diff --git a/deep-gan-encoders_amd/csrc/wgrad_dma.hip b/deep-gan-encoders_amd/csrc/wgrad_dma.hip
--- a/deep-gan-encoders_amd/csrc/wgrad_dma.hip
+++ b/deep-gan-encoders_amd/csrc/wgrad_dma.hip
@@ -23,18 +23,23 @@
 }
 constexpr unsigned DEAD = 0x7fffffffu;
 
-template <int TH_, int GP_, int XP_, int NW_, int NS_>
+template <int TH_, int GP_, int XP_, int NW_, int NS_, bool POOLED_ = false>
 struct WCfg {
     static constexpr int TH = TH_, GP = GP_, XP = XP_, NW = NW_, NS = NS_;
+    static constexpr bool POOLED = POOLED_;
     static constexpr int TW = 16, HH = TH + 2, HWD = TW + 2;
     static constexpr int GBYTES = TH * TW * GP;
     static constexpr int XBYTES = ((HH * HWD + 4) * XP + 1023) / 1024 * 1024;
-    static constexpr int NGP = GBYTES / 1024, NXP = XBYTES / 1024, NP = NGP + NXP;
+    static constexpr int NPP = GBYTES / 4096;
+    static constexpr int NGP = POOLED ? NPP + 1 : GBYTES / 1024, NXP = XBYTES / 1024, NP = NGP + NXP;
     static constexpr int PW = (NP + NW - 1) / NW;
-    static constexpr int STAGE = GBYTES + XBYTES;
+    static constexpr int STAGE = NGP * 1024 + XBYTES;
     static constexpr int RING = NS * STAGE;
+    static constexpr int GEXP_OFF = RING;
     static constexpr int FLUSH = (NW * 1024 + 1024 * 9) * 4;
-    static constexpr int MAIN = RING > FLUSH ? RING : FLUSH;
+    static constexpr int USED = RING + (POOLED ? GBYTES : 0);
+    static constexpr int MAIN = USED > FLUSH ? USED : FLUSH;
+    static_assert(!POOLED || (GP == 64 && GBYTES % 4096 == 0 && (TH / NW_) % 2 == 0 && (TH / 2) * 8 <= 64), "pooled form: 32-channel g slices, whole parent rows per wave");
     static constexpr int GTAB_OFF = MAIN, TAB_OFF = GTAB_OFF + 9 * 32 * 4;
     static constexpr int RW = TH / NW;
     static_assert(TH % NW == 0 && (NS - 2) * PW <= 63 && GBYTES % 1024 == 0 && NS >= 2 && NS <= 5, "configuration");
@@ -54,7 +59,8 @@
                                                                 const float* __restrict__ sc, const float* __restrict__ sh,
                                                                 float* __restrict__ dW, int B, int H, int W, int Co, int Ci,
                                                                 int tiles_x, int tiles_y, int per_group, int gps,
-                                                                const float* __restrict__ Wdot, float* __restrict__ dots, int dots_slots) {
+                                                                const float* __restrict__ Wdot, float* __restrict__ dots, int dots_slots,
+                                                                const unsigned* __restrict__ gmask, float gscale, float gslope) {
     constexpr int TH = C::TH, GP = C::GP, XP = C::XP, NW = C::NW, NS = C::NS, NT = NW * 64;
     extern __shared__ __attribute__((aligned(1024))) unsigned char lds[];
     float* gtab = (float*)(lds + C::GTAB_OFF);
@@ -87,12 +93,12 @@
         for (int r = 0; r < 16; r++) acc[t][r] = 0.f;
 
     constexpr int CG = GP / 16, CX = XP / 16, PPG = 1024 / GP, PPX = 1024 / XP;
-    constexpr int PG = C::NGP / NW, PX = (C::NXP + NW - 1) / NW;
-    static_assert(C::NGP % NW == 0 && PG + PX == C::PW, "piece split");
+    constexpr int PG = C::POOLED ? 1 : C::NGP / NW, PX = (C::NXP + NW - 1) / NW;
+    static_assert(C::POOLED || (C::NGP % NW == 0 && PG + PX == C::PW), "piece split");
     const int cg = lane % CG, pg = lane / CG, cx = lane % CX, px = lane / CX;
     const bool g_alive = o0 + cg * 8 < Co, x_alive = i0 + cx * 8 < Ci;
-    const bool last_x = wave + NW * (PX - 1) < C::NXP;
-    const int pw_mine = PG + PX - (last_x ? 0 : 1);
+    const bool last_x = C::POOLED ? wave + NW * (C::PW - 1) < C::NP : wave + NW * (PX - 1) < C::NXP;
+    const int pw_mine = C::POOLED ? C::PW - (last_x ? 0 : 1) : PG + PX - (last_x ? 0 : 1);
     unsigned rel_g[PG], rel_x[PX];
 #pragma unroll
     for (int j = 0; j < PG; j++) {
@@ -107,7 +113,55 @@
     const unsigned lds0 = lds_off(lds);
     const unsigned sample_g = (unsigned)H * W * Co * 2, sample_x = (unsigned)H * W * Ci * 2;
     int irem = t_begin - smp * tps, ity = irem / tiles_x, itx = irem - ity * tiles_x;
+    const int UW = W >> 1, UH = H >> 1, mwords = Co >> 3;
+    unsigned rel_p[C::POOLED ? C::PW : 1];
+    if constexpr (C::POOLED) {
+#pragma unroll
+        for (int j = 0; j < C::PW; j++) {
+            const int k = wave + NW * j;
+            if (k < C::NPP) {
+                const int q = k * 16 + (lane >> 2);
+                rel_p[j] = (unsigned)((((q >> 3) * UW + (q & 7)) * Co + o0 + (lane & 3) * 8) * 2);
+            } else if (k == C::NPP) {
+                rel_p[j] = lane < (TH / 2) * 8 ? (unsigned)((((lane >> 3) * UW + (lane & 7)) * mwords + (o0 >> 3)) * 4) : DEAD;
+            } else {
+                const int q = (k - C::NGP) * PPX + px, hy = q / C::HWD, hx = q - hy * C::HWD;
+                rel_p[j] = (q < C::HH * C::HWD && x_alive) ? (unsigned)((((hy - 1) * W + (hx - 1)) * Ci + i0 + cx * 8) * 2) : DEAD;
+            }
+        }
+    }
+    auto issue_pooled = [&](int stage) {
+        const unsigned m0w = lds0 + stage * C::STAGE + wave * 1024;
+        const int y0 = ity * TH, x0 = itx * 16;
+        const unsigned sample_p = (unsigned)UH * UW * Co * 2, sample_m = (unsigned)UH * UW * mwords * 4;
+        const rsrc_t rp = make_rsrc((unsigned long long)g + (unsigned long long)smp * sample_p, sample_p);
+        const rsrc_t rm = make_rsrc((unsigned long long)gmask + (unsigned long long)smp * sample_m, sample_m);
+        const rsrc_t rx = make_rsrc((unsigned long long)X + (unsigned long long)smp * sample_x, sample_x);
+        const unsigned par0 = (unsigned)((y0 >> 1) * UW + (x0 >> 1));
+        const unsigned pbase = par0 * (unsigned)Co * 2u, mbase = par0 * (unsigned)mwords * 4u, xbase = (unsigned)((y0 * W + x0) * Ci * 2);
+        const bool interior = (y0 >= 1) & (y0 + TH + 1 <= H) & (x0 >= 1) & (x0 + 17 <= W);
+#pragma unroll
+        for (int j = 0; j < C::PW; j++) {
+            if (j == C::PW - 1 && !last_x) break;
+            const int k = wave + NW * j;
+            const rsrc_t rs = k < C::NPP ? rp : (k == C::NPP ? rm : rx);
+            const unsigned base = k < C::NPP ? pbase : (k == C::NPP ? mbase : xbase);
+            bool ok = rel_p[j] != DEAD;
+            if (!interior) {
+                if (k <= C::NPP) {
+                    const int q = k < C::NPP ? k * 16 + (lane >> 2) : lane;
+                    ok = ok & ((y0 >> 1) + (q >> 3) < UH) & ((x0 >> 1) + (q & 7) < UW);
+                } else {
+                    const int q = (k - C::NGP) * PPX + px, hy = q / C::HWD, hx = q - hy * C::HWD;
+                    ok = ok & ((unsigned)(y0 + hy - 1) < (unsigned)H) & ((unsigned)(x0 + hx - 1) < (unsigned)W);
+                }
+            }
+            dma16(ok ? base + rel_p[j] : DEAD, rs, m0w + j * NW * 1024);
+        }
+        if (++itx == tiles_x) { itx = 0; ++ity; }
+    };
     auto issue = [&](int stage) {
+        if constexpr (C::POOLED) { issue_pooled(stage); return; }
         const unsigned mg = lds0 + stage * C::STAGE + wave * 1024, mx = mg + C::GBYTES;
         const int y0 = ity * TH, x0 = itx * 16;
         const rsrc_t rg = make_rsrc((unsigned long long)g + (unsigned long long)smp * sample_g, sample_g);
@@ -188,8 +242,29 @@
         DGE_WT(2);
         if (t + NS - 1 < t_end) issue(stage == 0 ? NS - 1 : stage - 1);
         DGE_WT(3);
-        const unsigned char* sg = lds + stage * C::STAGE;
-        const unsigned char* sx = sg + C::GBYTES;
+        const unsigned char* sg = C::POOLED ? lds + C::GEXP_OFF : lds + stage * C::STAGE;
+        const unsigned char* sx = lds + stage * C::STAGE + C::NGP * 1024;
+        if constexpr (C::POOLED) {
+            constexpr int UPW = (C::RW / 2) * 8 * 4;
+            if (lane < UPW) {
+                const unsigned char* st = lds + stage * C::STAGE;
+                const uint4 gv = *(const uint4*)(st + wave * (UPW * 16) + lane * 16);
+                const unsigned mw = *(const unsigned*)(st + C::NPP * 1024 + wave * (UPW * 4) + lane * 4);
+                float f[8];
+                unpack16(gv, f, (bf16_t*)nullptr);
+#pragma unroll
+                for (int e = 0; e < 8; e++) f[e] *= gscale;
+                const int ql = lane >> 2;
+                unsigned char* dst = lds + C::GEXP_OFF + ((C::RW * wave + 2 * (ql >> 3)) * 16 + 2 * (ql & 7)) * GP + (lane & 3) * 16;
+#pragma unroll
+                for (int c4 = 0; c4 < 4; c4++) {
+                    float o[8];
+#pragma unroll
+                    for (int e = 0; e < 8; e++) o[e] = f[e] * (((mw >> (c4 * 8 + e)) & 1u) ? 1.f : gslope);
+                    *(uint4*)(dst + ((c4 >> 1) * 16 + (c4 & 1)) * GP) = pack16(o, (bf16_t*)nullptr);
+                }
+            }
+        }
         const int y0 = cty * TH, x0 = ctx * 16;
         const bool edge_tile = (y0 == 0) | (y0 + TH >= H) | (x0 == 0) | (x0 + 16 >= W);
         uint4 av[2];
@@ -321,9 +396,11 @@
     }
 }
 
+struct PooledG { const unsigned* mask; float scale, slope; };
+
 template <class C>
 int launch(const void* g, const void* x, const float* sc, const float* sh, float* dw, int B, int H, int W, int cout, int cin,
-           const float* wdot, float* dots, int dots_slots, hipStream_t s) {
+           const float* wdot, float* dots, int dots_slots, hipStream_t s, PooledG pg = PooledG{nullptr, 1.f, 1.f}) {
     const int tx = (W + 15) / 16, ty = (H + C::TH - 1) / C::TH;
     const int tps = tx * ty;
     const int noi = ((cout + 31) / 32) * ((cin + 31) / 32);
@@ -349,9 +426,9 @@
     const int groups = B * gps;
     const int groups8 = groups < 8 ? groups : (groups + 7) / 8 * 8;
     if (!dge_det_fits(noi, (long long)B * gps, 1024 * 9)) return 1;
-    dge_note_kernel("wgrad_dma<%d,%d,%d,%d>", C::TH, C::GP, C::XP, C::NS);
+    dge_note_kernel(C::POOLED ? "wgrad_dma<%d,%d,%d,%d,pooled_g>" : "wgrad_dma<%d,%d,%d,%d>", C::TH, C::GP, C::XP, C::NS);
     hipLaunchKernelGGL(kern, dim3(noi, groups8), dim3(C::NW * 64), lds_bytes, s, (const bf16_t*)g, (const bf16_t*)x, sc, sh, dw, B, H, W,
-                       cout, cin, tx, ty, per, gps, wdot, dots, dots_slots < 1 ? 1 : dots_slots);
+                       cout, cin, tx, ty, per, gps, wdot, dots, dots_slots < 1 ? 1 : dots_slots, pg.mask, pg.scale, pg.slope);
     DGE_LAUNCH_CHECK("wgrad_dma");
     return 0;
 }
@@ -389,3 +466,20 @@
     if (cin <= 32 && cout <= 64) return launch<WCfg<8, 64, 64, 4, 3>>(g, x, sc, sh, dw, B, H, W, cout, cin, wdot, dots, dots_slots, s);
     return launch<WCfg<16, 64, 64, 4, 2>>(g, x, sc, sh, dw, B, H, W, cout, cin, wdot, dots, dots_slots, s);
 }
+
+bool dge_wgrad_dma_pooled_ok(int B, int H, int W, int cout, int cin) {
+    if (getenv("DGE_NO_WGRAD_DMA")) return false;
+    if (!(cout == 32 || cout == 64) || cin % 8 || cin > 32 || (H & 1) || (W & 1)) return false;
+    if ((size_t)H * W * cout * 2 >= (1u << 30) || (size_t)H * W * cin * 2 >= (1u << 30)) return false;
+    const int tps = ((W + 15) / 16) * ((H + 15) / 16);
+    const int noi = ((cout + 31) / 32) * ((cin + 31) / 32);
+    return tps >= 16 && noi * B <= 1024;
+}
+int dge_wgrad_dma_pooled_try(const void* gup, const unsigned* mask, float scale, float slope, const void* x, const float* sc, const float* sh,
+                             float* dw, int B, int H, int W, int cout, int cin, const float* wdot, float* dots, int dots_slots, hipStream_t s) {
+    if (!dge_wgrad_dma_pooled_ok(B, H, W, cout, cin)) return 1;
+    if (dots && (!sc || !wdot || !dge_det_fits(1LL << 40, 1, 1))) return 1;
+    const PooledG pg{mask, scale, slope};
+    if (cin <= 16) return launch<WCfg<16, 64, 32, 4, 3, true>>(gup, x, sc, sh, dw, B, H, W, cout, cin, wdot, dots, dots_slots, s, pg);
+    return launch<WCfg<8, 64, 64, 4, 4, true>>(gup, x, sc, sh, dw, B, H, W, cout, cin, wdot, dots, dots_slots, s, pg);
+}
diff --git a/deep-gan-encoders_amd/ops.py b/deep-gan-encoders_amd/ops.py
--- a/deep-gan-encoders_amd/ops.py
+++ b/deep-gan-encoders_amd/ops.py
@@ -329,6 +329,9 @@
         H, W = 2 * H, 2 * W
     if in_t2d:
         H, W = H - 1, W - 1
+    pooled_g = in_bwd.get("pooled") if in_bwd is not None else None
+    if pooled_g is not None:
+        H, W = 2 * H, 2 * W
     dt = dtype_of(x)
     OH, OW = (2 * H, 2 * W) if up else (H, W)
     mask = None
@@ -398,6 +401,10 @@
         d.stats_slots = max(1, min(64, nblk // 16))
         pn = in_bwd.get("noise")
         d.in_bwd_coef = _f32(in_bwd["coef"])
+        if pooled_g is not None:
+            if in_bwd.get("red") is None or in_bwd.get("fr") is not None:
+                raise DgeError("conv2d: a pooled input gradient goes with the activation form of in_bwd (red)")
+            d.pg_mask, d.pg_scale, d.pg_slope = _p(pooled_g["mask"]), float(pooled_g["scale"]), float(pooled_g.get("slope", 0.2))
         d.prep_noise, d.prep_noise_batch = _f32(pn), 1 if pn is None else pn.shape[0]
         if in_bwd.get("fr") is not None:
             d.fr_img4, d.in_bwd_extra, d.in_bwd_extra_scale = _f32(in_bwd["img4"]), _p(in_bwd.get("extra")), float(in_bwd.get("extra_scale", 1.0))
@@ -444,6 +451,10 @@
 
 def conv_in_bwd_supported(B, H, W, cin, cout, dtype):
     return bool(lib().dge_conv_in_bwd_supported(int(B), int(H), int(W), int(cin), int(cout), 3, int(dtype)))
+
+
+def conv_pooled_g_supported(B, H, W, cin, cout, dtype):
+    return bool(lib().dge_conv_pooled_g_supported(int(B), int(H), int(W), int(cin), int(cout), 3, int(dtype)))
 
 
 def conv_in_bwd_x_supported(B, H, W, cin, cout, dtype):
@@ -770,6 +781,22 @@
     return True
 
 
+def conv_wgrad_dots_pooled(gup, mask, scale, x, dw, in_scale, in_shift, w, dots, slope=0.2):
+    B, H, W, Cin = x.shape
+    cout = dw.shape[0]
+    if dw.shape[2] != 3 or is_deterministic():
+        return False
+    nslot = max(1, min(16, (H * W) // 4096))
+    buf = dots.alloc(nslot)
+    r = lib().dge_conv_wgrad_dots_pooled(_p(gup), _p(mask), float(scale), float(slope), _p(x), _f32(in_scale), _f32(in_shift), _f32(dw),
+                                         _f32(w.detach()), _f32(buf), nslot, B, H, W, cout, Cin, dtype_of(x), _stream())
+    if r == 1:
+        dots.buf, dots.nslot = None, 1
+        return False
+    check(r, "dge_conv_wgrad_dots_pooled")
+    return True
+
+
 class DeferredSums:
 
     def __init__(self):
@@ -813,10 +840,10 @@
     return gpre
 
 
-def act_bwd_mask(gup, mask, noise, scale=1.0, red=None, slope=0.2, planar=False, defer=None):
+def act_bwd_mask(gup, mask, noise, scale=1.0, red=None, slope=0.2, planar=False, defer=None, store=True):
     B, UH, UW, Cc = gup.shape
     H, W = 2 * UH, 2 * UW
-    gpre = torch.empty((B, H, W, Cc), dtype=gup.dtype, device=gup.device)
+    gpre = torch.empty((B, H, W, Cc), dtype=gup.dtype, device=gup.device) if store else None
     ncol = 2 if red is None else (red.shape[0] if planar else red.shape[-1])
     part = zeros((B, Cc, ncol), gup.device) if red is not None else None
     check(lib().dge_act_bwd_mask(_p(gup), _p(mask), _f32(noise), _p(gpre), _f32(part), ncol, B, H, W, Cc, float(scale), float(slope),
diff --git a/include/dge_hip.h b/include/dge_hip.h
--- a/include/dge_hip.h
+++ b/include/dge_hip.h
@@ -73,6 +73,8 @@
     float in_bwd_extra_scale;
     const float* fr_img4;
     float* fr_out;
+    const void* pg_mask;
+    float pg_scale, pg_slope;
 } dge_conv_desc;
 int dge_conv2d(const dge_conv_desc* d, dge_stream_t stream);
 int dge_conv_small_supported(int H, int W, int cin, int ntot, int ksize, int in_s2d, int in_up2, int dtype);
@@ -114,6 +116,7 @@
 int dge_conv_in_bwd_supported(int B, int H, int W, int Cin, int Cout, int ksize, int dtype);
 int dge_conv_in_bwd_fromrgb_supported(int B, int H, int W, int Cin, int Cout, int ksize, int dtype);
 int dge_conv_in_bwd_x_supported(int B, int H, int W, int Cin, int Cout, int ksize, int dtype);
+int dge_conv_pooled_g_supported(int B, int H, int W, int Cin, int Cout, int ksize, int dtype);
 int dge_conv_pool_supported(int B, int H, int W, int Cin, int Cout, int ksize, int dtype);
 int dge_rgb_upsample_add(float* img, const float* prev, int BC, int H, int W, dge_stream_t stream);
 int dge_nchw_to_nhwc(const float* src, void* dst, int B, int C, int HW, int src_B, int dtype, dge_stream_t stream);
@@ -189,6 +192,9 @@
                         float beta, int dtype, dge_stream_t stream);
 int dge_act_bwd_mask(const void* gup, const unsigned* mask, const float* noise, void* gpre, float* red, int red_cols, int B, int H, int W,
                      int C, float scale, float slope, int dtype, dge_stream_t stream);
+int dge_conv_wgrad_dots_pooled(const void* gup, const unsigned* mask, float scale, float slope, const void* x, const float* in_scale,
+                               const float* in_shift, float* dw, const float* w, float* dots, int dots_slots, int B, int H, int W,
+                               int cout, int cin, int dtype, dge_stream_t stream);
 int dge_fromrgb_dgrad(const void* gx, const void* x0, const float* w, float* gimg, int B, int HW, int C, int dtype, dge_stream_t stream);
 int dge_nearest_up2(const void* x, void* y, int B, int H, int W, int C, float scale, int dtype, dge_stream_t stream);
 int dge_in_bwd_coef(const float* dots, const float* gms, const float* musig, const float* sc, const float* sh, float* coef,
```

New measurement: 350.3 images/sec. 0.977x the previous value.
